# nv-nguyen/gigapose

Measured on NVIDIA H100. Metric: detections/sec (224x224 crops, 162-template bank), higher is better.
Workload: dtype f32 (a1, a4, a6: bf16 hi/lo split x3 on tensor cores with fp32 accumulate = fp32-faithful; a5, a7-a9: fp32)

## Files before the change

### gigapose_b200/csrc/gigapose_kernels.h

```cpp
#pragma once
#include <cuda_runtime.h>
#include <cuda.h>
#include <stdint.h>

namespace gp {

bool pdl_enabled();
template <typename... KArgs, typename... Args>
inline cudaError_t launch_ex(void (*kernel)(KArgs...), dim3 grid, dim3 block, size_t smem, cudaStream_t stream, int cluster_x,
                             bool pdl, Args&&... args) {
  cudaLaunchConfig_t cfg{};
  cfg.gridDim = grid; cfg.blockDim = block; cfg.dynamicSmemBytes = smem; cfg.stream = stream;
  cudaLaunchAttribute attr[2];
  int na = 0;
  if (cluster_x > 1) {
    attr[na].id = cudaLaunchAttributeClusterDimension;
    attr[na].val.clusterDim.x = cluster_x; attr[na].val.clusterDim.y = 1; attr[na].val.clusterDim.z = 1;
    ++na;
  }
  if (pdl && pdl_enabled()) {
    attr[na].id = cudaLaunchAttributeProgrammaticStreamSerialization;
    attr[na].val.programmaticStreamSerializationAllowed = 1;
    ++na;
  }
  cfg.attrs = attr; cfg.numAttrs = na;
  return cudaLaunchKernelEx(&cfg, kernel, static_cast<KArgs>(args)...);
}

struct SimSearchParams {
  int num_items;
  int B;
  int T;
  const int* perm;
  const int* q_obj;
  const float* q_mask;
  const float* bank_mask;
  float sim_threshold;
  float patch_threshold;
  int passes;
  float* sim_avg;
  float* rec_score;
  uint8_t* rec_idx;
  uint8_t* rec_valid;
  float* debug_tile;
};
cudaError_t launch_sim_search(const CUtensorMap& q_hi, const CUtensorMap& q_lo, const CUtensorMap& t_hi,
                              const CUtensorMap& t_lo, const SimSearchParams& p, int num_sms, cudaStream_t stream);
int sim_search_smem_bytes();

struct TopkSelectParams {
  int B, T, k;
  int id_stride, id_offset;
  const float* sim_avg;
  const float* rec_score;
  const uint8_t* rec_idx;
  const uint8_t* rec_valid;
  float* cand_score;
  int* cand_id;
  float* cand_pts_score;
  uint8_t* cand_idx;
  uint8_t* cand_valid;
};
cudaError_t launch_topk_select(const TopkSelectParams& p, cudaStream_t stream);

struct TopkMergeParams {
  int B, k, G;
  size_t rank_stride_bytes;
  const float* cand_score;
  const int* cand_id;
  const float* cand_pts_score;
  const uint8_t* cand_idx;
  const uint8_t* cand_valid;
  const float* cand_rel_scale;
  const float* cand_rel_inplane;
  float* out_rel_scale;
  float* out_rel_inplane;
  long long* id_src;
  float* score_src;
  float* score_pts;
  long long* tar_pts;
  long long* src_pts;
};
cudaError_t launch_topk_merge_expand(const TopkMergeParams& p, cudaStream_t stream);

cudaError_t launch_split_descriptors(const float* x, long long n_rows, int C, int rows_per_img, long long img_stride,
                                     long long row_stride, long long chan_stride, int norm_passes,
                                     int tiled ,
                                     uint16_t* hi, uint16_t* lo, float* normalized_out ,
                                     cudaStream_t stream);
cudaError_t launch_sample_mask16(const float* mask, long long n, int H, int W, float* out, cudaStream_t stream);
cudaError_t launch_object_order(const int* q_obj, int B, int num_objects, int* q_obj_out, int* perm, cudaStream_t stream);
cudaError_t launch_transpose_cp(const float* in, long long n, int C, float* out, cudaStream_t stream);

struct IstMlpWeights {
  const float *s_w1, *s_b1, *s_w2, *s_b2, *s_w3, *s_b3;
  const float *i_w1, *i_b1, *i_w2, *i_b2, *i_w3, *i_b3;
  int use_tanh;
};
struct IstMlpParams {
  int B, k;
  int T;
  int id_stride, id_offset;
  const long long* id_src;
  const long long* src_pts;
  const long long* tar_pts;
  const int* q_obj;
  const float* q_ist;
  const float* bank_ist;
  float* rel_scale;
  float* rel_inplane;
  int* row_count;
  int* row_ids;
  float* hidden1;
  float* hidden2;
};
cudaError_t launch_ist_mlp(const IstMlpWeights& w, const IstMlpParams& p, cudaStream_t stream);
cudaError_t launch_mlp_gather_planes(const IstMlpParams& p, uint16_t* a_hi, uint16_t* a_lo, cudaStream_t stream);
cudaError_t launch_mlp_head_rows(const IstMlpWeights& w, const IstMlpParams& p, const float* h2_scale, const float* h2_inplane,
                                 cudaStream_t stream);

struct RansacParams {
  int n;
  float pixel_threshold;
  int patch_size;
  const long long* src_pts;
  const long long* tar_pts;
  const float* rel_scale;
  const float* rel_inplane;
  float* M;
  uint8_t* failed;
  long long* in_src;
  long long* in_tar;
  long long* in_score;
  int* in_count;
};
cudaError_t launch_ransac(const RansacParams& p, cudaStream_t stream);

struct PoseParams {
  int B, k, T;
  int sort;
  const int* q_obj;
  const float* q_K;
  const float* q_M;
  const float* tmpl_K;
  const float* tmpl_M;
  const float* tmpl_pose;
  const int* in_count;
  const long long* id_src; const float* score_src; const float* score_pts;
  const long long* tar_pts; const long long* src_pts;
  const float* rel_scale; const float* rel_inplane;
  const float* M; const uint8_t* failed;
  const long long* in_src; const long long* in_tar; const long long* in_score;
  long long* o_id_src; float* o_score_src; float* o_score_pts;
  long long* o_tar_pts; long long* o_src_pts;
  float* o_rel_scale; float* o_rel_inplane;
  float* o_M; uint8_t* o_failed;
  long long* o_in_src; long long* o_in_tar; long long* o_in_score;
  float* o_scores;
  float* o_poses;
};
cudaError_t launch_sort_and_pose(const PoseParams& p, cudaStream_t stream);
cudaError_t launch_pose_only(int n, int k, int T, const int* q_obj, const float* q_K, const float* q_M,
                             const long long* id_src, const float* M, const float* tmpl_K, const float* tmpl_M,
                             const float* tmpl_pose, float* poses, cudaStream_t stream);

enum GemmMode { GEMM_PLANES = 0, GEMM_PLANES_GELU = 1, GEMM_SCALE_RESIDUAL = 2, GEMM_PATCH_EMBED = 3, GEMM_QKV_HEADS = 4,
                GEMM_PLANES_RELU = 5, GEMM_PLANES_ADD_RELU = 6, GEMM_ROWS_F32 = 7, GEMM_ROWS_F32_RELU = 8 };
struct GemmParams {
  int M, N, K;
  int passes;
  int mode;
  const float* bias;
  const float* gamma;
  float* x;
  uint16_t *out_hi, *out_lo;
  const float* pos;
  int tokens_per_img, patches_per_img;
  int qkv_crop_stride;
  int bn;
  int conv, Ho, Wo, stride, pad, kw, cblocks;
  int swap;
  const uint16_t *res_hi, *res_lo;
  const int* m_dev;
  float acc_scale;
  int f16;
  int stamp;
};
bool gemm_config_supported(const GemmParams& p, const char** why = nullptr);
cudaError_t launch_vit_gemm(const CUtensorMap& a_hi, const CUtensorMap& a_lo, const CUtensorMap& w_hi,
                            const CUtensorMap& w_lo, const GemmParams& p, int num_sms, cudaStream_t stream);
cudaError_t launch_split_planes(const float* x, long long rows, int K, int Kpad, uint16_t* hi, uint16_t* lo, cudaStream_t s,
                                bool f16 = false, float pre_scale = 1.0f);
cudaError_t launch_im2col(const float* img, int b, int Kpad, uint16_t* hi, uint16_t* lo, cudaStream_t s);
cudaError_t launch_cls_rows(const float* cls, const float* pos, int b, float* x, cudaStream_t s);
cudaError_t launch_layernorm_planes(const float* x, int M, const float* w, const float* b, float eps, uint16_t* hi,
                                    uint16_t* lo, cudaStream_t s);
cudaError_t launch_attention_tc(const CUtensorMap& hi128, const CUtensorMap& lo128, const CUtensorMap& hi16,
                                const CUtensorMap& lo16, const uint16_t* qkv_hi, const uint16_t* qkv_lo, uint16_t* out_hi,
                                uint16_t* out_lo, int b, int crop_stride, int passes, cudaStream_t s);
cudaError_t read_attention_stamps(long long* host32);
cudaError_t read_gemm_stamps(long long* host128);

}
```

### gigapose_b200/csrc/vit_api.cu

```cuda
#include "../../include/gigapose_b200.h"
#include "gigapose_kernels.h"

#include <cstdarg>
#include <cstdio>
#include <cstdlib>
#include <new>
#include <string>
#include <vector>

extern int gp_internal_fail(int code, const char* fmt, ...);
extern void gp_internal_count_launches(int n);
extern int gp_internal_make_map(CUtensorMap* map, void* ptr, uint64_t rows, uint64_t cols, uint32_t box_rows);
extern int gp_internal_make_map_ex(CUtensorMap* map, void* ptr, uint64_t rows, uint64_t cols, uint32_t box_cols,
                                   uint32_t box_rows, int swizzle_bytes);

namespace {

constexpr int kDim = 1024, kQkv = 3072, kMlp = 4096, kTok = 257, kPatchK = 588, kPatchKPad = 608;
constexpr float kLayerNormEps = 1e-6f;
constexpr size_t kAlign = 1024;
inline size_t up(size_t x) { return (x + kAlign - 1) / kAlign * kAlign; }

struct Carver {
  uint8_t* base; size_t off = 0;
  explicit Carver(void* b) : base(static_cast<uint8_t*>(b)) {}
  template <typename T> T* take(size_t n) { T* p = base ? reinterpret_cast<T*>(base + off) : nullptr; off += up(n * sizeof(T)); return p; }
};

struct Planes { uint16_t *hi, *lo; CUtensorMap m_hi, m_lo; };

struct BlockW {
  Planes qkv, proj, fc1, fc2;
  const float *n1w, *n1b, *qkv_b, *proj_b, *ls1, *n2w, *n2b, *fc1_b, *fc2_b, *ls2;
};

#define GPV_CUDA(expr)                                                                                    \
  do {                                                                                                    \
    cudaError_t _e = (expr);                                                                              \
    if (_e != cudaSuccess) return gp_internal_fail(GP_ERR_CUDA, "%s failed: %s", #expr, cudaGetErrorString(_e)); \
  } while (0)

}

struct gp_vit_context {
  int depth, max_crops, passes, num_sms;
  Planes patch_w;
  const float *patch_b, *cls, *pos;
  std::vector<BlockW> blocks;
  float* x;
  Planes ln, qkv, attn, hid, patches;
  CUtensorMap qkv_hi128, qkv_lo128, qkv_hi16, qkv_lo16;
  size_t workspace_bytes;
};

namespace {

void carve_weights(Carver& c, int depth, gp_vit_context* h) {
  auto planes = [&](Planes* p, size_t n) { uint16_t* a = c.take<uint16_t>(n); uint16_t* b = c.take<uint16_t>(n); if (p) { p->hi = a; p->lo = b; } };
  planes(h ? &h->patch_w : nullptr, (size_t)kDim * kPatchKPad);
  for (int i = 0; i < depth; ++i) {
    BlockW* b = h ? &h->blocks[i] : nullptr;
    planes(b ? &b->qkv : nullptr, (size_t)kQkv * kDim);
    planes(b ? &b->proj : nullptr, (size_t)kDim * kDim);
    planes(b ? &b->fc1 : nullptr, (size_t)kMlp * kDim);
    planes(b ? &b->fc2 : nullptr, (size_t)kDim * kMlp);
  }
}

void carve_workspace(Carver& c, int max_crops, gp_vit_context* h) {
  const size_t M = (size_t)max_crops * kTok;
  auto planes = [&](Planes* p, size_t n) { uint16_t* a = c.take<uint16_t>(n); uint16_t* b = c.take<uint16_t>(n); if (p) { p->hi = a; p->lo = b; } };
  float* x = c.take<float>(M * kDim);
  if (h) h->x = x;
  planes(h ? &h->ln : nullptr, M * kDim);
  planes(h ? &h->qkv : nullptr, M * kQkv);
  planes(h ? &h->attn : nullptr, M * kDim);
  planes(h ? &h->hid : nullptr, M * kMlp);
  planes(h ? &h->patches : nullptr, (size_t)max_crops * 256 * kPatchKPad);
}

int make_maps(Planes* p, uint64_t rows, uint64_t cols, uint32_t box_rows) {
  if (int e = gp_internal_make_map(&p->m_hi, p->hi, rows, cols, box_rows)) return e;
  return gp_internal_make_map(&p->m_lo, p->lo, rows, cols, box_rows);
}

}

extern "C" {

int gp_vit_query_sizes(int depth, int max_crops, size_t* weight_bytes, size_t* workspace_bytes) {
  if (depth < 1 || depth > 64 || max_crops < 1) return gp_internal_fail(GP_ERR_INVALID, "bad depth / max_crops");
  Carver cw(nullptr), cs(nullptr);
  carve_weights(cw, depth, nullptr);
  carve_workspace(cs, max_crops, nullptr);
  if (weight_bytes) *weight_bytes = cw.off;
  if (workspace_bytes) *workspace_bytes = cs.off;
  return GP_OK;
}

int gp_vit_create(int device, int depth, int max_crops, int precision, const float* const* w, void* weight_mem,
                  void* workspace_mem, void* stream, gp_vit_handle_t* out) {
  if (depth < 1 || depth > 64 || max_crops < 1 || !w || !weight_mem || !workspace_mem || !out)
    return gp_internal_fail(GP_ERR_INVALID, "bad argument");
  if (precision != GP_PRECISION_FP32_SPLIT && precision != GP_PRECISION_BF16)
    return gp_internal_fail(GP_ERR_INVALID, "unknown precision %d", precision);
  if (((uintptr_t)weight_mem | (uintptr_t)workspace_mem) & (kAlign - 1))
    return gp_internal_fail(GP_ERR_INVALID, "weight and workspace memory must be 1024-byte aligned");
  for (int i = 0; i < 4 + 14 * depth; ++i)
    if (!w[i]) return gp_internal_fail(GP_ERR_INVALID, "weight pointer %d is null", i);
  GPV_CUDA(cudaSetDevice(device));
  cudaDeviceProp prop;
  GPV_CUDA(cudaGetDeviceProperties(&prop, device));
  if (prop.major != 9 || prop.minor != 0) return gp_internal_fail(GP_ERR_UNSUPPORTED, "device %d is not sm_90", device);
  gp_vit_context* h = new (std::nothrow) gp_vit_context();
  if (!h) return gp_internal_fail(GP_ERR_INVALID, "out of host memory");
  h->depth = depth; h->max_crops = max_crops; h->num_sms = prop.multiProcessorCount;
  h->passes = precision == GP_PRECISION_FP32_SPLIT ? 3 : 1;
  h->blocks.resize(depth);
  Carver cw(weight_mem), cs(workspace_mem);
  carve_weights(cw, depth, h);
  carve_workspace(cs, max_crops, h);
  cudaStream_t s = static_cast<cudaStream_t>(stream);
  if (cudaMemsetAsync(workspace_mem, 0, cs.off, s) != cudaSuccess) { delete h; return gp_internal_fail(GP_ERR_CUDA, "workspace memset failed"); }

  h->patch_b = w[1]; h->cls = w[2]; h->pos = w[3];
  cudaError_t ce = gp::launch_split_planes(w[0], kDim, kPatchK, kPatchKPad, h->patch_w.hi, h->patch_w.lo, s);
  int e = ce == cudaSuccess ? make_maps(&h->patch_w, kDim, kPatchKPad, 256) : GP_ERR_CUDA;
  for (int i = 0; i < depth && !e && ce == cudaSuccess; ++i) {
    const float* const* b = w + 4 + 14 * i;
    BlockW& B = h->blocks[i];
    B.n1w = b[0]; B.n1b = b[1]; B.qkv_b = b[3]; B.proj_b = b[5]; B.ls1 = b[6];
    B.n2w = b[7]; B.n2b = b[8]; B.fc1_b = b[10]; B.fc2_b = b[12]; B.ls2 = b[13];
    if ((ce = gp::launch_split_planes(b[2], kQkv, kDim, kDim, B.qkv.hi, B.qkv.lo, s)) != cudaSuccess) break;
    if ((ce = gp::launch_split_planes(b[4], kDim, kDim, kDim, B.proj.hi, B.proj.lo, s)) != cudaSuccess) break;
    if ((ce = gp::launch_split_planes(b[9], kMlp, kDim, kDim, B.fc1.hi, B.fc1.lo, s)) != cudaSuccess) break;
    if ((ce = gp::launch_split_planes(b[11], kDim, kMlp, kMlp, B.fc2.hi, B.fc2.lo, s)) != cudaSuccess) break;
    if ((e = make_maps(&B.qkv, kQkv, kDim, 256)) || (e = make_maps(&B.proj, kDim, kDim, 256)) ||
        (e = make_maps(&B.fc1, kMlp, kDim, 256)) || (e = make_maps(&B.fc2, kDim, kMlp, 256)))
      break;
  }
  const uint64_t M = (uint64_t)max_crops * kTok;
  if (!e && ce == cudaSuccess)
    (e = make_maps(&h->ln, M, kDim, 128)) || (e = make_maps(&h->attn, M, kDim, 128)) || (e = make_maps(&h->hid, M, kMlp, 128)) ||
        (e = make_maps(&h->patches, (uint64_t)max_crops * 256, kPatchKPad, 128)) ||
        (e = gp_internal_make_map_ex(&h->qkv_hi128, h->qkv.hi, 48 * M, 64, 64, 128, 128)) ||
        (e = gp_internal_make_map_ex(&h->qkv_lo128, h->qkv.lo, 48 * M, 64, 64, 128, 128)) ||
        (e = gp_internal_make_map_ex(&h->qkv_hi16, h->qkv.hi, 48 * M, 64, 64, 16, 128)) ||
        (e = gp_internal_make_map_ex(&h->qkv_lo16, h->qkv.lo, 48 * M, 64, 64, 16, 128));
  if (ce != cudaSuccess) { delete h; return gp_internal_fail(GP_ERR_CUDA, "weight packing failed: %s", cudaGetErrorString(ce)); }
  if (e) { delete h; return e; }
  gp_internal_count_launches(1 + 4 * depth);
  *out = h;
  return GP_OK;
}

int gp_debug_attention_timeline(long long* stamps32) {
  if (!stamps32) return gp_internal_fail(GP_ERR_INVALID, "null argument");
  GPV_CUDA(cudaDeviceSynchronize());
  GPV_CUDA(gp::read_attention_stamps(stamps32));
  return GP_OK;
}

int gp_debug_gemm_timeline(long long* stamps128) {
  if (!stamps128) return gp_internal_fail(GP_ERR_INVALID, "null argument");
  GPV_CUDA(cudaDeviceSynchronize());
  GPV_CUDA(gp::read_gemm_stamps(stamps128));
  return GP_OK;
}

int gp_debug_gemm(const gp_debug_gemm_t* d, void* stream) {
  if (!d) return gp_internal_fail(GP_ERR_INVALID, "null argument");
  gp::GemmParams g{};
  g.M = d->M; g.N = d->N; g.K = d->K; g.bn = d->bn; g.passes = d->passes; g.mode = d->mode; g.swap = d->swap; g.f16 = d->f16;
  g.acc_scale = d->acc_scale; g.bias = d->bias; g.gamma = d->gamma; g.x = d->x; g.out_hi = d->out_hi; g.out_lo = d->out_lo;
  g.pos = d->pos; g.res_hi = d->res_hi; g.res_lo = d->res_lo; g.m_dev = d->m_dev;
  g.tokens_per_img = d->tokens_per_img; g.patches_per_img = d->patches_per_img; g.qkv_crop_stride = d->qkv_crop_stride;
  g.stamp = d->stamp;
  if (g.M < 1) return gp_internal_fail(GP_ERR_INVALID, "M must be >= 1");
  const char* why = nullptr;
  if (!gp::gemm_config_supported(g, &why)) return gp_internal_fail(GP_ERR_INVALID, "unsupported GEMM: %s", why);
  if (!d->a_hi || !d->a_lo || !d->w_hi || !d->w_lo || !d->bias) return gp_internal_fail(GP_ERR_INVALID, "null operand or bias");
  const bool planes_out = g.mode == gp::GEMM_PLANES || g.mode == gp::GEMM_PLANES_GELU || g.mode == gp::GEMM_QKV_HEADS ||
                          g.mode == gp::GEMM_PLANES_RELU || g.mode == gp::GEMM_PLANES_ADD_RELU;
  if (planes_out ? (!g.out_hi || !g.out_lo) : !g.x) return gp_internal_fail(GP_ERR_INVALID, "null output");
  if (g.mode == gp::GEMM_SCALE_RESIDUAL && !g.gamma) return gp_internal_fail(GP_ERR_INVALID, "null gamma");
  if (g.mode == gp::GEMM_PLANES_ADD_RELU && (!g.res_hi || !g.res_lo)) return gp_internal_fail(GP_ERR_INVALID, "null residual planes");
  if (g.mode == gp::GEMM_PATCH_EMBED && (!g.pos || g.patches_per_img < 1 || g.tokens_per_img <= g.patches_per_img))
    return gp_internal_fail(GP_ERR_INVALID, "patch embedding needs pos and tokens_per_img > patches_per_img >= 1");
  if (g.mode == gp::GEMM_QKV_HEADS && (g.N != kQkv || g.tokens_per_img < 1 || g.qkv_crop_stride * g.tokens_per_img < g.M))
    return gp_internal_fail(GP_ERR_INVALID, "QKV scatter needs N = 3072 and qkv_crop_stride * tokens_per_img >= M");
  if (g.swap && g.m_dev) return gp_internal_fail(GP_ERR_INVALID, "m_dev is not supported with swap");
  int dev = 0, sms = 0;
  GPV_CUDA(cudaGetDevice(&dev));
  GPV_CUDA(cudaDeviceGetAttribute(&sms, cudaDevAttrMultiProcessorCount, dev));
  const int bn = g.bn > 0 ? g.bn : 256;
  CUtensorMap a_hi, a_lo, w_hi, w_lo;
  auto* a_h = const_cast<uint16_t*>(d->a_hi); auto* a_l = const_cast<uint16_t*>(d->a_lo);
  auto* w_h = const_cast<uint16_t*>(d->w_hi); auto* w_l = const_cast<uint16_t*>(d->w_lo);
  if (int e = gp_internal_make_map(&a_hi, a_h, g.M, g.K, 128)) return e;
  if (int e = gp_internal_make_map(&a_lo, a_l, g.M, g.K, 128)) return e;
  if (int e = gp_internal_make_map(&w_hi, w_h, g.N, g.K, bn)) return e;
  if (int e = gp_internal_make_map(&w_lo, w_l, g.N, g.K, bn)) return e;
  GPV_CUDA(gp::launch_vit_gemm(a_hi, a_lo, w_hi, w_lo, g, sms, static_cast<cudaStream_t>(stream)));
  gp_internal_count_launches(1);
  return GP_OK;
}

int gp_debug_attention(int b, int crop_stride, int passes, const uint16_t* qkv_hi, const uint16_t* qkv_lo, uint16_t* out_hi,
                       uint16_t* out_lo, void* stream) {
  if (!qkv_hi || !qkv_lo || !out_hi || !out_lo) return gp_internal_fail(GP_ERR_INVALID, "null argument");
  if (b < 1 || crop_stride < b) return gp_internal_fail(GP_ERR_INVALID, "need 1 <= b (%d) <= crop_stride (%d)", b, crop_stride);
  if (passes != 1 && passes != 3) return gp_internal_fail(GP_ERR_INVALID, "passes must be 1 or 3");
  const uint64_t rows = 48ull * crop_stride * kTok;
  auto* qh = const_cast<uint16_t*>(qkv_hi); auto* ql = const_cast<uint16_t*>(qkv_lo);
  CUtensorMap hi128, lo128, hi16, lo16;
  if (int e = gp_internal_make_map_ex(&hi128, qh, rows, 64, 64, 128, 128)) return e;
  if (int e = gp_internal_make_map_ex(&lo128, ql, rows, 64, 64, 128, 128)) return e;
  if (int e = gp_internal_make_map_ex(&hi16, qh, rows, 64, 64, 16, 128)) return e;
  if (int e = gp_internal_make_map_ex(&lo16, ql, rows, 64, 64, 16, 128)) return e;
  GPV_CUDA(gp::launch_attention_tc(hi128, lo128, hi16, lo16, qkv_hi, qkv_lo, out_hi, out_lo, b, crop_stride, passes,
                                   static_cast<cudaStream_t>(stream)));
  gp_internal_count_launches(1);
  return GP_OK;
}

int gp_debug_layernorm(int M, const float* x, const float* w, const float* b, uint16_t* out_hi, uint16_t* out_lo,
                       void* stream) {
  if (!x || !w || !b || !out_hi || !out_lo) return gp_internal_fail(GP_ERR_INVALID, "null argument");
  if (M < 1) return gp_internal_fail(GP_ERR_INVALID, "M must be >= 1");
  GPV_CUDA(gp::launch_layernorm_planes(x, M, w, b, kLayerNormEps, out_hi, out_lo, static_cast<cudaStream_t>(stream)));
  gp_internal_count_launches(1);
  return GP_OK;
}

int gp_vit_destroy(gp_vit_handle_t h) {
  delete h;
  return GP_OK;
}

int gp_vit_time_linears(gp_vit_handle_t h, int b, int iters, float* avg_ms, void* stream) {
  if (!h || !avg_ms || iters < 1) return gp_internal_fail(GP_ERR_INVALID, "bad argument");
  if (b < 1 || b > h->max_crops) return gp_internal_fail(GP_ERR_INVALID, "batch %d outside [1, %d]", b, h->max_crops);
  cudaStream_t s = static_cast<cudaStream_t>(stream);
  const int M = b * kTok;
  auto linear = [&](const Planes& a, const Planes& w, gp::GemmParams& gp_) {
    return gp::launch_vit_gemm(a.m_hi, a.m_lo, w.m_hi, w.m_lo, gp_, h->num_sms, s);
  };
  auto run = [&]() -> int {
    for (int i = 0; i < h->depth; ++i) {
      const BlockW& B = h->blocks[i];
      gp::GemmParams g{};
      g.passes = h->passes; g.M = M; g.N = kQkv; g.K = kDim; g.mode = gp::GEMM_QKV_HEADS; g.bias = B.qkv_b;
      g.out_hi = h->qkv.hi; g.out_lo = h->qkv.lo; g.tokens_per_img = kTok; g.qkv_crop_stride = h->max_crops;
      GPV_CUDA(linear(h->ln, B.qkv, g));
      g = gp::GemmParams{}; g.passes = h->passes;
      g.M = M; g.N = kDim; g.K = kDim; g.mode = gp::GEMM_SCALE_RESIDUAL; g.bias = B.proj_b; g.gamma = B.ls1; g.x = h->x;
      GPV_CUDA(linear(h->attn, B.proj, g));
      g = gp::GemmParams{}; g.passes = h->passes;
      g.M = M; g.N = kMlp; g.K = kDim; g.mode = gp::GEMM_PLANES_GELU; g.bias = B.fc1_b; g.out_hi = h->hid.hi; g.out_lo = h->hid.lo;
      GPV_CUDA(linear(h->ln, B.fc1, g));
      g = gp::GemmParams{}; g.passes = h->passes;
      g.M = M; g.N = kDim; g.K = kMlp; g.mode = gp::GEMM_SCALE_RESIDUAL; g.bias = B.fc2_b; g.gamma = B.ls2; g.x = h->x;
      GPV_CUDA(linear(h->hid, B.fc2, g));
    }
    return GP_OK;
  };
  cudaEvent_t e0, e1;
  GPV_CUDA(cudaEventCreate(&e0));
  GPV_CUDA(cudaEventCreate(&e1));
  if (int e = run()) return e;
  GPV_CUDA(cudaEventRecord(e0, s));
  for (int it = 0; it < iters; ++it)
    if (int e = run()) return e;
  GPV_CUDA(cudaEventRecord(e1, s));
  GPV_CUDA(cudaEventSynchronize(e1));
  float ms = 0.f;
  GPV_CUDA(cudaEventElapsedTime(&ms, e0, e1));
  cudaEventDestroy(e0);
  cudaEventDestroy(e1);
  *avg_ms = ms / iters;
  gp_internal_count_launches(4 * h->depth * (iters + 1));
  return GP_OK;
}

int gp_vit_forward(gp_vit_handle_t h, int b, const float* img, float* x_prenorm, void* stream) {
  if (!h || !img || !x_prenorm) return gp_internal_fail(GP_ERR_INVALID, "null argument");
  if (b < 1 || b > h->max_crops) return gp_internal_fail(GP_ERR_INVALID, "batch %d outside [1, %d]", b, h->max_crops);
  cudaStream_t s = static_cast<cudaStream_t>(stream);
  const int M = b * kTok;
  GPV_CUDA(gp::launch_im2col(img, b, kPatchKPad, h->patches.hi, h->patches.lo, s));
  gp::GemmParams g{};
  g.passes = h->passes; g.tokens_per_img = kTok; g.patches_per_img = 256;
  g.M = b * 256; g.N = kDim; g.K = kPatchKPad; g.mode = gp::GEMM_PATCH_EMBED; g.bias = h->patch_b; g.pos = h->pos; g.x = h->x;
  GPV_CUDA(gp::launch_vit_gemm(h->patches.m_hi, h->patches.m_lo, h->patch_w.m_hi, h->patch_w.m_lo, g, h->num_sms, s));
  GPV_CUDA(gp::launch_cls_rows(h->cls, h->pos, b, h->x, s));
  auto linear = [&](const Planes& a, const Planes& w, gp::GemmParams& gp_) {
    return gp::launch_vit_gemm(a.m_hi, a.m_lo, w.m_hi, w.m_lo, gp_, h->num_sms, s);
  };
  for (int i = 0; i < h->depth; ++i) {
    const BlockW& B = h->blocks[i];
    GPV_CUDA(gp::launch_layernorm_planes(h->x, M, B.n1w, B.n1b, kLayerNormEps, h->ln.hi, h->ln.lo, s));
    g = gp::GemmParams{}; g.passes = h->passes;
    g.M = M; g.N = kQkv; g.K = kDim; g.mode = gp::GEMM_QKV_HEADS; g.bias = B.qkv_b; g.out_hi = h->qkv.hi; g.out_lo = h->qkv.lo;
    g.tokens_per_img = kTok; g.qkv_crop_stride = h->max_crops;
    GPV_CUDA(linear(h->ln, B.qkv, g));
    GPV_CUDA(gp::launch_attention_tc(h->qkv_hi128, h->qkv_lo128, h->qkv_hi16, h->qkv_lo16, h->qkv.hi, h->qkv.lo,
                                     h->attn.hi, h->attn.lo, b, h->max_crops, h->passes, s));
    g = gp::GemmParams{}; g.passes = h->passes;
    g.M = M; g.N = kDim; g.K = kDim; g.mode = gp::GEMM_SCALE_RESIDUAL; g.bias = B.proj_b; g.gamma = B.ls1; g.x = h->x;
    GPV_CUDA(linear(h->attn, B.proj, g));
    GPV_CUDA(gp::launch_layernorm_planes(h->x, M, B.n2w, B.n2b, kLayerNormEps, h->ln.hi, h->ln.lo, s));
    g = gp::GemmParams{}; g.passes = h->passes;
    g.M = M; g.N = kMlp; g.K = kDim; g.mode = gp::GEMM_PLANES_GELU; g.bias = B.fc1_b; g.out_hi = h->hid.hi; g.out_lo = h->hid.lo;
    GPV_CUDA(linear(h->ln, B.fc1, g));
    g = gp::GemmParams{}; g.passes = h->passes;
    g.M = M; g.N = kDim; g.K = kMlp; g.mode = gp::GEMM_SCALE_RESIDUAL; g.bias = B.fc2_b; g.gamma = B.ls2; g.x = h->x;
    GPV_CUDA(linear(h->hid, B.fc2, g));
  }
  GPV_CUDA(cudaMemcpyAsync(x_prenorm, h->x, (size_t)M * kDim * sizeof(float), cudaMemcpyDeviceToDevice, s));
  gp_internal_count_launches(3 + 7 * h->depth);
  return GP_OK;
}

}
```

### gigapose_b200/csrc/vit_attention_tc.cu

```cuda
#include "gigapose_kernels.h"
#include "common.cuh"
#include "wgmma.cuh"
#include <cuda_bf16.h>

namespace gp {

namespace {

constexpr int kTok = 257, kDim = 1024, kHeads = 16, kHd = 64;
constexpr int kKeys = 272;
constexpr int kRow = 128;
constexpr int kKVPlane = kKeys * kRow;
constexpr int kQPlane = 256 * kRow;
constexpr int kQTiles = 4;
constexpr int kMmaWarps = 8;
constexpr int kThreads = (kMmaWarps + 1) * 32;

struct __align__(8) AttnTail {
  uint64_t qk_full, v_full;
};
constexpr int kSmem = 1024 + 4 * kKVPlane + 2 * kQPlane + sizeof(AttnTail);

__device__ __forceinline__ void split_pair(float a, float b, uint32_t& hi, uint32_t& lo) {
  asm("cvt.rn.bf16x2.f32 %0, %1, %2;" : "=r"(hi) : "f"(b), "f"(a));
  const float ra = a - __uint_as_float(hi << 16), rb = b - __uint_as_float(hi & 0xffff0000u);
  asm("cvt.rn.bf16x2.f32 %0, %1, %2;" : "=r"(lo) : "f"(rb), "f"(ra));
}
__device__ __forceinline__ float ex2_approx(float x) {
  float y;
  asm("ex2.approx.ftz.f32 %0, %1;" : "=f"(y) : "f"(x));
  return y;
}
constexpr float kExpScale = 0.125f * 1.4426950408889634f;
__device__ __forceinline__ float2 ld_pair_sw128(const uint8_t* hi, const uint8_t* lo, int row, int col) {
  const uint32_t off = (uint32_t)row * 128u + ((((uint32_t)col >> 3) ^ ((uint32_t)row & 7u)) << 4) + (((uint32_t)col & 7u) << 1);
  const uint32_t h = *reinterpret_cast<const uint32_t*>(hi + off);
  const uint32_t l = lo ? *reinterpret_cast<const uint32_t*>(lo + off) : 0u;
  return make_float2(__uint_as_float(h << 16) + __uint_as_float(l << 16),
                     __uint_as_float(h & 0xffff0000u) + __uint_as_float(l & 0xffff0000u));
}

}

__device__ long long g_attn_stamp[32];
#define STAMP(i) do { if (blockIdx.x == 0) g_attn_stamp[i] = clock64(); } while (0)

template <int kPasses>
__global__ void __launch_bounds__(kThreads, 1)
attention_tc_kernel(const __grid_constant__ CUtensorMap tm_hi_128, const __grid_constant__ CUtensorMap tm_lo_128,
                    const __grid_constant__ CUtensorMap tm_hi_16, const __grid_constant__ CUtensorMap tm_lo_16,
                    const __nv_bfloat16* __restrict__ qkv_hi, const __nv_bfloat16* __restrict__ qkv_lo,
                    __nv_bfloat16* __restrict__ out_hi, __nv_bfloat16* __restrict__ out_lo, int crop_stride) {
  constexpr int passes = kPasses;
  constexpr int np = passes == 3 ? 2 : 1;
  extern __shared__ uint8_t smem_raw[];
  pdl_trigger();
  uint8_t* smem = smem_raw + ((1024u - (smem_u32(smem_raw) & 1023u)) & 1023u);
  uint8_t* sK[2] = {smem, smem + kKVPlane};
  uint8_t* sV[2] = {smem + 2 * kKVPlane, smem + 3 * kKVPlane};
  uint8_t* sQ[2] = {smem + 4 * kKVPlane, smem + 4 * kKVPlane + kQPlane};
  AttnTail& tail = *reinterpret_cast<AttnTail*>(smem + 4 * kKVPlane + 2 * kQPlane);
  const int warp = threadIdx.x >> 5, lane = threadIdx.x & 31;
  const int item = blockIdx.x;
  const int img = item / kHeads, head = item % kHeads;
  const int row0 = img * kTok;
  const int rq = ((0 * crop_stride + img) * kHeads + head) * kTok;
  const int rk = ((1 * crop_stride + img) * kHeads + head) * kTok;
  const int rv = ((2 * crop_stride + img) * kHeads + head) * kTok;

  if (threadIdx.x == 0) {
    mbar_init(&tail.qk_full, 1);
    mbar_init(&tail.v_full, 1);
    fence_barrier_init();
  }
  __syncthreads();
  pdl_wait();
  if (threadIdx.x == 0) STAMP(0);

  if (warp == kMmaWarps) {
    if (lane == 0) {
      tma_prefetch_desc(&tm_hi_128); tma_prefetch_desc(&tm_hi_16);
      if (np == 2) { tma_prefetch_desc(&tm_lo_128); tma_prefetch_desc(&tm_lo_16); }
      mbar_arrive_expect_tx(&tail.qk_full, (uint32_t)(np * (kQPlane + kKVPlane)));
      for (int pl = 0; pl < np; ++pl) {
        const CUtensorMap* m128 = pl ? &tm_lo_128 : &tm_hi_128;
        const CUtensorMap* m16 = pl ? &tm_lo_16 : &tm_hi_16;
        tma_load_2d(sQ[pl], m128, &tail.qk_full, 0, rq);
        tma_load_2d(sQ[pl] + 128 * kRow, m128, &tail.qk_full, 0, rq + 128);
        tma_load_2d(sK[pl], m128, &tail.qk_full, 0, rk);
        tma_load_2d(sK[pl] + 128 * kRow, m128, &tail.qk_full, 0, rk + 128);
        tma_load_2d(sK[pl] + 256 * kRow, m16, &tail.qk_full, 0, rk + 256);
      }
      mbar_arrive_expect_tx(&tail.v_full, (uint32_t)(np * kKVPlane));
      for (int pl = 0; pl < np; ++pl) {
        const CUtensorMap* m128 = pl ? &tm_lo_128 : &tm_hi_128;
        const CUtensorMap* m16 = pl ? &tm_lo_16 : &tm_hi_16;
        tma_load_2d(sV[pl], m128, &tail.v_full, 0, rv);
        tma_load_2d(sV[pl] + 128 * kRow, m128, &tail.v_full, 0, rv + 128);
        tma_load_2d(sV[pl] + 256 * kRow, m16, &tail.v_full, 0, rv + 256);
      }
    }
    __syncwarp();
    __shared__ float s_p[kKeys];
    __shared__ float s_q[kHd];
    {
    const size_t qoff = (size_t)(rq + 256) * kHd + 2 * lane;
    const uint32_t qh = *reinterpret_cast<const uint32_t*>(qkv_hi + qoff);
    const uint32_t ql = passes == 3 ? *reinterpret_cast<const uint32_t*>(qkv_lo + qoff) : 0u;
    s_q[2 * lane] = __uint_as_float(qh << 16) + __uint_as_float(ql << 16);
    s_q[2 * lane + 1] = __uint_as_float(qh & 0xffff0000u) + __uint_as_float(ql & 0xffff0000u);
    __syncwarp();
    mbar_wait(&tail.qk_full, 0);
    const uint8_t* klo = passes == 3 ? sK[1] : nullptr;
    const uint8_t* vlo = passes == 3 ? sV[1] : nullptr;
    float sj[9];
    float mx = -INFINITY;
#pragma unroll
    for (int i = 0; i < 9; ++i) {
      const int key = lane + 32 * i;
      float acc = 0.f;
      if (key < kTok) {
#pragma unroll
        for (int ch = 0; ch < 8; ++ch) {
          const uint32_t off = (uint32_t)key * 128u + (((uint32_t)ch ^ ((uint32_t)key & 7u)) << 4);
          const uint4 h4 = *reinterpret_cast<const uint4*>(sK[0] + off);
          const uint4 l4 = klo ? *reinterpret_cast<const uint4*>(klo + off) : make_uint4(0, 0, 0, 0);
          const uint32_t hw[4] = {h4.x, h4.y, h4.z, h4.w}, lw[4] = {l4.x, l4.y, l4.z, l4.w};
#pragma unroll
          for (int w = 0; w < 4; ++w) {
            const float k0 = __uint_as_float(hw[w] << 16) + __uint_as_float(lw[w] << 16);
            const float k1 = __uint_as_float(hw[w] & 0xffff0000u) + __uint_as_float(lw[w] & 0xffff0000u);
            acc = fmaf(s_q[ch * 8 + 2 * w], k0, acc);
            acc = fmaf(s_q[ch * 8 + 2 * w + 1], k1, acc);
          }
        }
      }
      sj[i] = key < kTok ? acc : -INFINITY;
      mx = fmaxf(mx, sj[i]);
    }
#pragma unroll
    for (int off = 16; off > 0; off >>= 1) mx = fmaxf(mx, __shfl_xor_sync(0xffffffffu, mx, off));
    float sum = 0.f;
#pragma unroll
    for (int i = 0; i < 9; ++i) {
      const int key = lane + 32 * i;
      const float pj = key < kTok ? ex2_approx((sj[i] - mx) * kExpScale) : 0.f;
      sum += pj;
      if (key < kKeys) s_p[key] = pj;
    }
#pragma unroll
    for (int off = 16; off > 0; off >>= 1) sum += __shfl_xor_sync(0xffffffffu, sum, off);
    __syncwarp();
    mbar_wait(&tail.v_full, 0);
    float o0[4] = {0.f, 0.f, 0.f, 0.f}, o1[4] = {0.f, 0.f, 0.f, 0.f};
#pragma unroll 8
    for (int key = 0; key < 256; ++key) {
      const float2 vv = ld_pair_sw128(sV[0], vlo, key, 2 * lane);
      const float pj = s_p[key];
      o0[key & 3] = fmaf(pj, vv.x, o0[key & 3]);
      o1[key & 3] = fmaf(pj, vv.y, o1[key & 3]);
    }
    {
      const float2 vv = ld_pair_sw128(sV[0], vlo, 256, 2 * lane);
      o0[0] = fmaf(s_p[256], vv.x, o0[0]);
      o1[0] = fmaf(s_p[256], vv.y, o1[0]);
    }
    const float o0s = (o0[0] + o0[1]) + (o0[2] + o0[3]), o1s = (o1[0] + o1[1]) + (o1[2] + o1[3]);
    const float inv = 1.0f / sum;
    uint32_t h, l;
    split_pair(o0s * inv, o1s * inv, h, l);
    const size_t oo = (size_t)(row0 + 256) * kDim + head * kHd + 2 * lane;
    *reinterpret_cast<uint32_t*>(out_hi + oo) = h;
    *reinterpret_cast<uint32_t*>(out_lo + oo) = l;
    }
  } else {
    const int wg = warp >> 2, wl = warp & 3;
    const uint32_t kh = smem_u32(sK[0]), kl = smem_u32(sK[1]), vh = smem_u32(sV[0]), vl = smem_u32(sV[1]);
    mbar_wait(&tail.qk_full, 0);
    if (threadIdx.x == 0) STAMP(1);
    for (int qt = wg; qt < kQTiles; qt += 2) {
      const uint32_t qh = smem_u32(sQ[0] + qt * 64 * kRow), ql = smem_u32(sQ[1] + qt * 64 * kRow);
      float s[128], st[8];
      acc_fence(s); acc_fence(st);
      wgmma_fence();
#pragma unroll
      for (int pass = 0; pass < passes; ++pass) {
        const uint32_t a = pass == 2 ? ql : qh, b = pass == 1 ? kl : kh;
#pragma unroll
        for (int k16 = 0; k16 < 4; ++k16) {
          const uint32_t acc = (pass | k16) != 0 ? 1u : 0u;
          const uint64_t da = wgmma_desc_kmajor<kRow>(a + k16 * 32);
          wgmma_ss_n256_bf16(s, da, wgmma_desc_kmajor<kRow>(b + k16 * 32), acc);
          wgmma_ss_n16_bf16(st, da, wgmma_desc_kmajor<kRow>(b + 256 * kRow + k16 * 32), acc);
        }
      }
      wgmma_commit();
      wgmma_wait<0>();
      acc_fence(s); acc_fence(st);
      const bool key256 = (lane & 3) == 0;
#pragma unroll
      for (int i = 0; i < 8; ++i) if (!(key256 && (i & 1) == 0 && i < 4)) st[i] = -INFINITY;
      float mx0 = fmaxf(st[0], st[1]), mx1 = fmaxf(st[2], st[3]);
#pragma unroll
      for (int j = 0; j < 32; ++j) {
        mx0 = fmaxf(mx0, fmaxf(s[4 * j], s[4 * j + 1]));
        mx1 = fmaxf(mx1, fmaxf(s[4 * j + 2], s[4 * j + 3]));
      }
#pragma unroll
      for (int off = 1; off <= 2; off <<= 1) {
        mx0 = fmaxf(mx0, __shfl_xor_sync(0xffffffffu, mx0, off));
        mx1 = fmaxf(mx1, __shfl_xor_sync(0xffffffffu, mx1, off));
      }
      float sum0 = 0.f, sum1 = 0.f;
      uint32_t ph[68], pl[68];
#pragma unroll
      for (int j = 0; j < 34; ++j) {
        const float x0 = j < 32 ? s[4 * j] : st[4 * (j - 32)], x1 = j < 32 ? s[4 * j + 1] : st[4 * (j - 32) + 1];
        const float x2 = j < 32 ? s[4 * j + 2] : st[4 * (j - 32) + 2], x3 = j < 32 ? s[4 * j + 3] : st[4 * (j - 32) + 3];
        const float p0 = ex2_approx((x0 - mx0) * kExpScale), p1 = ex2_approx((x1 - mx0) * kExpScale);
        const float p2 = ex2_approx((x2 - mx1) * kExpScale), p3 = ex2_approx((x3 - mx1) * kExpScale);
        sum0 += p0 + p1;
        sum1 += p2 + p3;
        const int c = j >> 1, h = (j & 1) * 2;
        split_pair(p0, p1, ph[4 * c + h], pl[4 * c + h]);
        split_pair(p2, p3, ph[4 * c + h + 1], pl[4 * c + h + 1]);
      }
#pragma unroll
      for (int off = 1; off <= 2; off <<= 1) {
        sum0 += __shfl_xor_sync(0xffffffffu, sum0, off);
        sum1 += __shfl_xor_sync(0xffffffffu, sum1, off);
      }
      if (qt == wg) mbar_wait(&tail.v_full, 0);
      float o[32];
      acc_fence(o);
      wgmma_fence();
#pragma unroll
      for (int c = 0; c < kKeys / 16; ++c) {
        const uint32_t ah[4] = {ph[4 * c], ph[4 * c + 1], ph[4 * c + 2], ph[4 * c + 3]};
        const uint64_t dvh = wgmma_desc_mnmajor_sw128(vh + c * 16 * kRow);
        wgmma_rs_n64_bf16_tb(o, ah, dvh, c != 0 ? 1u : 0u);
        if (passes == 3) {
          const uint32_t al[4] = {pl[4 * c], pl[4 * c + 1], pl[4 * c + 2], pl[4 * c + 3]};
          wgmma_rs_n64_bf16_tb(o, ah, wgmma_desc_mnmajor_sw128(vl + c * 16 * kRow), 1u);
          wgmma_rs_n64_bf16_tb(o, al, dvh, 1u);
        }
      }
      wgmma_commit();
      wgmma_wait<0>();
      acc_fence(o);
      const float inv0 = 1.0f / sum0, inv1 = 1.0f / sum1;
      const int tok0 = qt * 64 + wl * 16 + (lane >> 2);
      const size_t o0 = (size_t)(row0 + tok0) * kDim + head * kHd + 2 * (lane & 3);
      const size_t o1 = o0 + (size_t)8 * kDim;
#pragma unroll
      for (int j = 0; j < 8; ++j) {
        uint32_t h, l;
        split_pair(o[4 * j] * inv0, o[4 * j + 1] * inv0, h, l);
        *reinterpret_cast<uint32_t*>(out_hi + o0 + 8 * j) = h;
        *reinterpret_cast<uint32_t*>(out_lo + o0 + 8 * j) = l;
        split_pair(o[4 * j + 2] * inv1, o[4 * j + 3] * inv1, h, l);
        *reinterpret_cast<uint32_t*>(out_hi + o1 + 8 * j) = h;
        *reinterpret_cast<uint32_t*>(out_lo + o1 + 8 * j) = l;
      }
    }
    if (lane == 0 && wl == 0) STAMP(2 + wg);
  }
}

cudaError_t read_attention_stamps(long long* host32) {
  return cudaMemcpyFromSymbol(host32, g_attn_stamp, sizeof(long long) * 32);
}

cudaError_t launch_attention_tc(const CUtensorMap& hi128, const CUtensorMap& lo128, const CUtensorMap& hi16,
                                const CUtensorMap& lo16, const uint16_t* qkv_hi, const uint16_t* qkv_lo, uint16_t* out_hi,
                                uint16_t* out_lo, int b, int crop_stride, int passes, cudaStream_t s) {
  static bool configured = false;
  if (!configured) {
    cudaError_t e = cudaFuncSetAttribute(attention_tc_kernel<3>, cudaFuncAttributeMaxDynamicSharedMemorySize, kSmem);
    if (e == cudaSuccess) e = cudaFuncSetAttribute(attention_tc_kernel<1>, cudaFuncAttributeMaxDynamicSharedMemorySize, kSmem);
    if (e != cudaSuccess) return e;
    configured = true;
  }
  if (b <= 0) return cudaSuccess;
  const int items = b * kHeads;
  const dim3 grid(items);
  auto qh = reinterpret_cast<const __nv_bfloat16*>(qkv_hi), ql = reinterpret_cast<const __nv_bfloat16*>(qkv_lo);
  auto oh = reinterpret_cast<__nv_bfloat16*>(out_hi), ol = reinterpret_cast<__nv_bfloat16*>(out_lo);
  if (passes == 3)
    return launch_ex(attention_tc_kernel<3>, grid, dim3(kThreads), kSmem, s, 1, true, hi128, lo128, hi16, lo16, qh, ql, oh, ol, crop_stride);
  return launch_ex(attention_tc_kernel<1>, grid, dim3(kThreads), kSmem, s, 1, true, hi128, lo128, hi16, lo16, qh, ql, oh, ol, crop_stride);
}

}
```

### gigapose_b200/csrc/wgmma.cuh

```cuda
#pragma once
#include <stdint.h>

namespace gp {

__device__ __forceinline__ void wgmma_ss_n16_bf16(float (&d)[8], uint64_t da, uint64_t db, uint32_t scale_d) {
  asm volatile(
      "{\n\t.reg .pred p;\n\t"
      "setp.ne.b32 p, %10, 0;\n\t"
      "wgmma.mma_async.sync.aligned.m64n16k16.f32.bf16.bf16 "
      "{%0, %1, %2, %3, %4, %5, %6, %7}, "
      "%8, %9, p, 1, 1, 0, 0;\n\t}"
      : "+f"(d[0]), "+f"(d[1]), "+f"(d[2]), "+f"(d[3]), "+f"(d[4]), "+f"(d[5]), "+f"(d[6]), "+f"(d[7])
      : "l"(da), "l"(db), "r"(scale_d));
}
__device__ __forceinline__ void wgmma_ss_n16_f16(float (&d)[8], uint64_t da, uint64_t db, uint32_t scale_d) {
  asm volatile(
      "{\n\t.reg .pred p;\n\t"
      "setp.ne.b32 p, %10, 0;\n\t"
      "wgmma.mma_async.sync.aligned.m64n16k16.f32.f16.f16 "
      "{%0, %1, %2, %3, %4, %5, %6, %7}, "
      "%8, %9, p, 1, 1, 0, 0;\n\t}"
      : "+f"(d[0]), "+f"(d[1]), "+f"(d[2]), "+f"(d[3]), "+f"(d[4]), "+f"(d[5]), "+f"(d[6]), "+f"(d[7])
      : "l"(da), "l"(db), "r"(scale_d));
}
__device__ __forceinline__ void wgmma_ss_n64_bf16(float (&d)[32], uint64_t da, uint64_t db, uint32_t scale_d) {
  asm volatile(
      "{\n\t.reg .pred p;\n\t"
      "setp.ne.b32 p, %34, 0;\n\t"
      "wgmma.mma_async.sync.aligned.m64n64k16.f32.bf16.bf16 "
      "{%0, %1, %2, %3, %4, %5, %6, %7, %8, %9, %10, %11, %12, %13, %14, %15, %16, %17, %18, %19, %20, %21, %22, %23, %24, %25, %26, %27, %28, %29, %30, %31}, "
      "%32, %33, p, 1, 1, 0, 0;\n\t}"
      : "+f"(d[0]), "+f"(d[1]), "+f"(d[2]), "+f"(d[3]), "+f"(d[4]), "+f"(d[5]), "+f"(d[6]), "+f"(d[7]), "+f"(d[8]), "+f"(d[9]), "+f"(d[10]), "+f"(d[11]), "+f"(d[12]), "+f"(d[13]), "+f"(d[14]), "+f"(d[15]), "+f"(d[16]), "+f"(d[17]), "+f"(d[18]), "+f"(d[19]), "+f"(d[20]), "+f"(d[21]), "+f"(d[22]), "+f"(d[23]), "+f"(d[24]), "+f"(d[25]), "+f"(d[26]), "+f"(d[27]), "+f"(d[28]), "+f"(d[29]), "+f"(d[30]), "+f"(d[31])
      : "l"(da), "l"(db), "r"(scale_d));
}
__device__ __forceinline__ void wgmma_ss_n64_f16(float (&d)[32], uint64_t da, uint64_t db, uint32_t scale_d) {
  asm volatile(
      "{\n\t.reg .pred p;\n\t"
      "setp.ne.b32 p, %34, 0;\n\t"
      "wgmma.mma_async.sync.aligned.m64n64k16.f32.f16.f16 "
      "{%0, %1, %2, %3, %4, %5, %6, %7, %8, %9, %10, %11, %12, %13, %14, %15, %16, %17, %18, %19, %20, %21, %22, %23, %24, %25, %26, %27, %28, %29, %30, %31}, "
      "%32, %33, p, 1, 1, 0, 0;\n\t}"
      : "+f"(d[0]), "+f"(d[1]), "+f"(d[2]), "+f"(d[3]), "+f"(d[4]), "+f"(d[5]), "+f"(d[6]), "+f"(d[7]), "+f"(d[8]), "+f"(d[9]), "+f"(d[10]), "+f"(d[11]), "+f"(d[12]), "+f"(d[13]), "+f"(d[14]), "+f"(d[15]), "+f"(d[16]), "+f"(d[17]), "+f"(d[18]), "+f"(d[19]), "+f"(d[20]), "+f"(d[21]), "+f"(d[22]), "+f"(d[23]), "+f"(d[24]), "+f"(d[25]), "+f"(d[26]), "+f"(d[27]), "+f"(d[28]), "+f"(d[29]), "+f"(d[30]), "+f"(d[31])
      : "l"(da), "l"(db), "r"(scale_d));
}
__device__ __forceinline__ void wgmma_ss_n192_bf16(float (&d)[96], uint64_t da, uint64_t db, uint32_t scale_d) {
  asm volatile(
      "{\n\t.reg .pred p;\n\t"
      "setp.ne.b32 p, %98, 0;\n\t"
      "wgmma.mma_async.sync.aligned.m64n192k16.f32.bf16.bf16 "
      "{%0, %1, %2, %3, %4, %5, %6, %7, %8, %9, %10, %11, %12, %13, %14, %15, %16, %17, %18, %19, %20, %21, %22, %23, %24, %25, %26, %27, %28, %29, %30, %31, %32, %33, %34, %35, %36, %37, %38, %39, %40, %41, %42, %43, %44, %45, %46, %47, %48, %49, %50, %51, %52, %53, %54, %55, %56, %57, %58, %59, %60, %61, %62, %63, %64, %65, %66, %67, %68, %69, %70, %71, %72, %73, %74, %75, %76, %77, %78, %79, %80, %81, %82, %83, %84, %85, %86, %87, %88, %89, %90, %91, %92, %93, %94, %95}, "
      "%96, %97, p, 1, 1, 0, 0;\n\t}"
      : "+f"(d[0]), "+f"(d[1]), "+f"(d[2]), "+f"(d[3]), "+f"(d[4]), "+f"(d[5]), "+f"(d[6]), "+f"(d[7]), "+f"(d[8]), "+f"(d[9]), "+f"(d[10]), "+f"(d[11]), "+f"(d[12]), "+f"(d[13]), "+f"(d[14]), "+f"(d[15]), "+f"(d[16]), "+f"(d[17]), "+f"(d[18]), "+f"(d[19]), "+f"(d[20]), "+f"(d[21]), "+f"(d[22]), "+f"(d[23]), "+f"(d[24]), "+f"(d[25]), "+f"(d[26]), "+f"(d[27]), "+f"(d[28]), "+f"(d[29]), "+f"(d[30]), "+f"(d[31]), "+f"(d[32]), "+f"(d[33]), "+f"(d[34]), "+f"(d[35]), "+f"(d[36]), "+f"(d[37]), "+f"(d[38]), "+f"(d[39]), "+f"(d[40]), "+f"(d[41]), "+f"(d[42]), "+f"(d[43]), "+f"(d[44]), "+f"(d[45]), "+f"(d[46]), "+f"(d[47]), "+f"(d[48]), "+f"(d[49]), "+f"(d[50]), "+f"(d[51]), "+f"(d[52]), "+f"(d[53]), "+f"(d[54]), "+f"(d[55]), "+f"(d[56]), "+f"(d[57]), "+f"(d[58]), "+f"(d[59]), "+f"(d[60]), "+f"(d[61]), "+f"(d[62]), "+f"(d[63]), "+f"(d[64]), "+f"(d[65]), "+f"(d[66]), "+f"(d[67]), "+f"(d[68]), "+f"(d[69]), "+f"(d[70]), "+f"(d[71]), "+f"(d[72]), "+f"(d[73]), "+f"(d[74]), "+f"(d[75]), "+f"(d[76]), "+f"(d[77]), "+f"(d[78]), "+f"(d[79]), "+f"(d[80]), "+f"(d[81]), "+f"(d[82]), "+f"(d[83]), "+f"(d[84]), "+f"(d[85]), "+f"(d[86]), "+f"(d[87]), "+f"(d[88]), "+f"(d[89]), "+f"(d[90]), "+f"(d[91]), "+f"(d[92]), "+f"(d[93]), "+f"(d[94]), "+f"(d[95])
      : "l"(da), "l"(db), "r"(scale_d));
}
__device__ __forceinline__ void wgmma_ss_n192_f16(float (&d)[96], uint64_t da, uint64_t db, uint32_t scale_d) {
  asm volatile(
      "{\n\t.reg .pred p;\n\t"
      "setp.ne.b32 p, %98, 0;\n\t"
      "wgmma.mma_async.sync.aligned.m64n192k16.f32.f16.f16 "
      "{%0, %1, %2, %3, %4, %5, %6, %7, %8, %9, %10, %11, %12, %13, %14, %15, %16, %17, %18, %19, %20, %21, %22, %23, %24, %25, %26, %27, %28, %29, %30, %31, %32, %33, %34, %35, %36, %37, %38, %39, %40, %41, %42, %43, %44, %45, %46, %47, %48, %49, %50, %51, %52, %53, %54, %55, %56, %57, %58, %59, %60, %61, %62, %63, %64, %65, %66, %67, %68, %69, %70, %71, %72, %73, %74, %75, %76, %77, %78, %79, %80, %81, %82, %83, %84, %85, %86, %87, %88, %89, %90, %91, %92, %93, %94, %95}, "
      "%96, %97, p, 1, 1, 0, 0;\n\t}"
      : "+f"(d[0]), "+f"(d[1]), "+f"(d[2]), "+f"(d[3]), "+f"(d[4]), "+f"(d[5]), "+f"(d[6]), "+f"(d[7]), "+f"(d[8]), "+f"(d[9]), "+f"(d[10]), "+f"(d[11]), "+f"(d[12]), "+f"(d[13]), "+f"(d[14]), "+f"(d[15]), "+f"(d[16]), "+f"(d[17]), "+f"(d[18]), "+f"(d[19]), "+f"(d[20]), "+f"(d[21]), "+f"(d[22]), "+f"(d[23]), "+f"(d[24]), "+f"(d[25]), "+f"(d[26]), "+f"(d[27]), "+f"(d[28]), "+f"(d[29]), "+f"(d[30]), "+f"(d[31]), "+f"(d[32]), "+f"(d[33]), "+f"(d[34]), "+f"(d[35]), "+f"(d[36]), "+f"(d[37]), "+f"(d[38]), "+f"(d[39]), "+f"(d[40]), "+f"(d[41]), "+f"(d[42]), "+f"(d[43]), "+f"(d[44]), "+f"(d[45]), "+f"(d[46]), "+f"(d[47]), "+f"(d[48]), "+f"(d[49]), "+f"(d[50]), "+f"(d[51]), "+f"(d[52]), "+f"(d[53]), "+f"(d[54]), "+f"(d[55]), "+f"(d[56]), "+f"(d[57]), "+f"(d[58]), "+f"(d[59]), "+f"(d[60]), "+f"(d[61]), "+f"(d[62]), "+f"(d[63]), "+f"(d[64]), "+f"(d[65]), "+f"(d[66]), "+f"(d[67]), "+f"(d[68]), "+f"(d[69]), "+f"(d[70]), "+f"(d[71]), "+f"(d[72]), "+f"(d[73]), "+f"(d[74]), "+f"(d[75]), "+f"(d[76]), "+f"(d[77]), "+f"(d[78]), "+f"(d[79]), "+f"(d[80]), "+f"(d[81]), "+f"(d[82]), "+f"(d[83]), "+f"(d[84]), "+f"(d[85]), "+f"(d[86]), "+f"(d[87]), "+f"(d[88]), "+f"(d[89]), "+f"(d[90]), "+f"(d[91]), "+f"(d[92]), "+f"(d[93]), "+f"(d[94]), "+f"(d[95])
      : "l"(da), "l"(db), "r"(scale_d));
}
__device__ __forceinline__ void wgmma_ss_n256_bf16(float (&d)[128], uint64_t da, uint64_t db, uint32_t scale_d) {
  asm volatile(
      "{\n\t.reg .pred p;\n\t"
      "setp.ne.b32 p, %130, 0;\n\t"
      "wgmma.mma_async.sync.aligned.m64n256k16.f32.bf16.bf16 "
      "{%0, %1, %2, %3, %4, %5, %6, %7, %8, %9, %10, %11, %12, %13, %14, %15, %16, %17, %18, %19, %20, %21, %22, %23, %24, %25, %26, %27, %28, %29, %30, %31, %32, %33, %34, %35, %36, %37, %38, %39, %40, %41, %42, %43, %44, %45, %46, %47, %48, %49, %50, %51, %52, %53, %54, %55, %56, %57, %58, %59, %60, %61, %62, %63, %64, %65, %66, %67, %68, %69, %70, %71, %72, %73, %74, %75, %76, %77, %78, %79, %80, %81, %82, %83, %84, %85, %86, %87, %88, %89, %90, %91, %92, %93, %94, %95, %96, %97, %98, %99, %100, %101, %102, %103, %104, %105, %106, %107, %108, %109, %110, %111, %112, %113, %114, %115, %116, %117, %118, %119, %120, %121, %122, %123, %124, %125, %126, %127}, "
      "%128, %129, p, 1, 1, 0, 0;\n\t}"
      : "+f"(d[0]), "+f"(d[1]), "+f"(d[2]), "+f"(d[3]), "+f"(d[4]), "+f"(d[5]), "+f"(d[6]), "+f"(d[7]), "+f"(d[8]), "+f"(d[9]), "+f"(d[10]), "+f"(d[11]), "+f"(d[12]), "+f"(d[13]), "+f"(d[14]), "+f"(d[15]), "+f"(d[16]), "+f"(d[17]), "+f"(d[18]), "+f"(d[19]), "+f"(d[20]), "+f"(d[21]), "+f"(d[22]), "+f"(d[23]), "+f"(d[24]), "+f"(d[25]), "+f"(d[26]), "+f"(d[27]), "+f"(d[28]), "+f"(d[29]), "+f"(d[30]), "+f"(d[31]), "+f"(d[32]), "+f"(d[33]), "+f"(d[34]), "+f"(d[35]), "+f"(d[36]), "+f"(d[37]), "+f"(d[38]), "+f"(d[39]), "+f"(d[40]), "+f"(d[41]), "+f"(d[42]), "+f"(d[43]), "+f"(d[44]), "+f"(d[45]), "+f"(d[46]), "+f"(d[47]), "+f"(d[48]), "+f"(d[49]), "+f"(d[50]), "+f"(d[51]), "+f"(d[52]), "+f"(d[53]), "+f"(d[54]), "+f"(d[55]), "+f"(d[56]), "+f"(d[57]), "+f"(d[58]), "+f"(d[59]), "+f"(d[60]), "+f"(d[61]), "+f"(d[62]), "+f"(d[63]), "+f"(d[64]), "+f"(d[65]), "+f"(d[66]), "+f"(d[67]), "+f"(d[68]), "+f"(d[69]), "+f"(d[70]), "+f"(d[71]), "+f"(d[72]), "+f"(d[73]), "+f"(d[74]), "+f"(d[75]), "+f"(d[76]), "+f"(d[77]), "+f"(d[78]), "+f"(d[79]), "+f"(d[80]), "+f"(d[81]), "+f"(d[82]), "+f"(d[83]), "+f"(d[84]), "+f"(d[85]), "+f"(d[86]), "+f"(d[87]), "+f"(d[88]), "+f"(d[89]), "+f"(d[90]), "+f"(d[91]), "+f"(d[92]), "+f"(d[93]), "+f"(d[94]), "+f"(d[95]), "+f"(d[96]), "+f"(d[97]), "+f"(d[98]), "+f"(d[99]), "+f"(d[100]), "+f"(d[101]), "+f"(d[102]), "+f"(d[103]), "+f"(d[104]), "+f"(d[105]), "+f"(d[106]), "+f"(d[107]), "+f"(d[108]), "+f"(d[109]), "+f"(d[110]), "+f"(d[111]), "+f"(d[112]), "+f"(d[113]), "+f"(d[114]), "+f"(d[115]), "+f"(d[116]), "+f"(d[117]), "+f"(d[118]), "+f"(d[119]), "+f"(d[120]), "+f"(d[121]), "+f"(d[122]), "+f"(d[123]), "+f"(d[124]), "+f"(d[125]), "+f"(d[126]), "+f"(d[127])
      : "l"(da), "l"(db), "r"(scale_d));
}
__device__ __forceinline__ void wgmma_ss_n256_f16(float (&d)[128], uint64_t da, uint64_t db, uint32_t scale_d) {
  asm volatile(
      "{\n\t.reg .pred p;\n\t"
      "setp.ne.b32 p, %130, 0;\n\t"
      "wgmma.mma_async.sync.aligned.m64n256k16.f32.f16.f16 "
      "{%0, %1, %2, %3, %4, %5, %6, %7, %8, %9, %10, %11, %12, %13, %14, %15, %16, %17, %18, %19, %20, %21, %22, %23, %24, %25, %26, %27, %28, %29, %30, %31, %32, %33, %34, %35, %36, %37, %38, %39, %40, %41, %42, %43, %44, %45, %46, %47, %48, %49, %50, %51, %52, %53, %54, %55, %56, %57, %58, %59, %60, %61, %62, %63, %64, %65, %66, %67, %68, %69, %70, %71, %72, %73, %74, %75, %76, %77, %78, %79, %80, %81, %82, %83, %84, %85, %86, %87, %88, %89, %90, %91, %92, %93, %94, %95, %96, %97, %98, %99, %100, %101, %102, %103, %104, %105, %106, %107, %108, %109, %110, %111, %112, %113, %114, %115, %116, %117, %118, %119, %120, %121, %122, %123, %124, %125, %126, %127}, "
      "%128, %129, p, 1, 1, 0, 0;\n\t}"
      : "+f"(d[0]), "+f"(d[1]), "+f"(d[2]), "+f"(d[3]), "+f"(d[4]), "+f"(d[5]), "+f"(d[6]), "+f"(d[7]), "+f"(d[8]), "+f"(d[9]), "+f"(d[10]), "+f"(d[11]), "+f"(d[12]), "+f"(d[13]), "+f"(d[14]), "+f"(d[15]), "+f"(d[16]), "+f"(d[17]), "+f"(d[18]), "+f"(d[19]), "+f"(d[20]), "+f"(d[21]), "+f"(d[22]), "+f"(d[23]), "+f"(d[24]), "+f"(d[25]), "+f"(d[26]), "+f"(d[27]), "+f"(d[28]), "+f"(d[29]), "+f"(d[30]), "+f"(d[31]), "+f"(d[32]), "+f"(d[33]), "+f"(d[34]), "+f"(d[35]), "+f"(d[36]), "+f"(d[37]), "+f"(d[38]), "+f"(d[39]), "+f"(d[40]), "+f"(d[41]), "+f"(d[42]), "+f"(d[43]), "+f"(d[44]), "+f"(d[45]), "+f"(d[46]), "+f"(d[47]), "+f"(d[48]), "+f"(d[49]), "+f"(d[50]), "+f"(d[51]), "+f"(d[52]), "+f"(d[53]), "+f"(d[54]), "+f"(d[55]), "+f"(d[56]), "+f"(d[57]), "+f"(d[58]), "+f"(d[59]), "+f"(d[60]), "+f"(d[61]), "+f"(d[62]), "+f"(d[63]), "+f"(d[64]), "+f"(d[65]), "+f"(d[66]), "+f"(d[67]), "+f"(d[68]), "+f"(d[69]), "+f"(d[70]), "+f"(d[71]), "+f"(d[72]), "+f"(d[73]), "+f"(d[74]), "+f"(d[75]), "+f"(d[76]), "+f"(d[77]), "+f"(d[78]), "+f"(d[79]), "+f"(d[80]), "+f"(d[81]), "+f"(d[82]), "+f"(d[83]), "+f"(d[84]), "+f"(d[85]), "+f"(d[86]), "+f"(d[87]), "+f"(d[88]), "+f"(d[89]), "+f"(d[90]), "+f"(d[91]), "+f"(d[92]), "+f"(d[93]), "+f"(d[94]), "+f"(d[95]), "+f"(d[96]), "+f"(d[97]), "+f"(d[98]), "+f"(d[99]), "+f"(d[100]), "+f"(d[101]), "+f"(d[102]), "+f"(d[103]), "+f"(d[104]), "+f"(d[105]), "+f"(d[106]), "+f"(d[107]), "+f"(d[108]), "+f"(d[109]), "+f"(d[110]), "+f"(d[111]), "+f"(d[112]), "+f"(d[113]), "+f"(d[114]), "+f"(d[115]), "+f"(d[116]), "+f"(d[117]), "+f"(d[118]), "+f"(d[119]), "+f"(d[120]), "+f"(d[121]), "+f"(d[122]), "+f"(d[123]), "+f"(d[124]), "+f"(d[125]), "+f"(d[126]), "+f"(d[127])
      : "l"(da), "l"(db), "r"(scale_d));
}
__device__ __forceinline__ void wgmma_rs_n64_bf16_tb(float (&d)[32], const uint32_t (&a)[4], uint64_t db, uint32_t scale_d) {
  asm volatile(
      "{\n\t.reg .pred p;\n\t"
      "setp.ne.b32 p, %37, 0;\n\t"
      "wgmma.mma_async.sync.aligned.m64n64k16.f32.bf16.bf16 "
      "{%0, %1, %2, %3, %4, %5, %6, %7, %8, %9, %10, %11, %12, %13, %14, %15, %16, %17, %18, %19, %20, %21, %22, %23, %24, %25, %26, %27, %28, %29, %30, %31}, "
      "{%32, %33, %34, %35}, %36, p, 1, 1, 1;\n\t}"
      : "+f"(d[0]), "+f"(d[1]), "+f"(d[2]), "+f"(d[3]), "+f"(d[4]), "+f"(d[5]), "+f"(d[6]), "+f"(d[7]), "+f"(d[8]), "+f"(d[9]), "+f"(d[10]), "+f"(d[11]), "+f"(d[12]), "+f"(d[13]), "+f"(d[14]), "+f"(d[15]), "+f"(d[16]), "+f"(d[17]), "+f"(d[18]), "+f"(d[19]), "+f"(d[20]), "+f"(d[21]), "+f"(d[22]), "+f"(d[23]), "+f"(d[24]), "+f"(d[25]), "+f"(d[26]), "+f"(d[27]), "+f"(d[28]), "+f"(d[29]), "+f"(d[30]), "+f"(d[31])
      : "r"(a[0]), "r"(a[1]), "r"(a[2]), "r"(a[3]), "l"(db), "r"(scale_d));
}

__device__ __forceinline__ void wgmma_fence() { asm volatile("wgmma.fence.sync.aligned;" ::: "memory"); }
__device__ __forceinline__ void wgmma_commit() { asm volatile("wgmma.commit_group.sync.aligned;" ::: "memory"); }
template <int kPending>
__device__ __forceinline__ void wgmma_wait() { asm volatile("wgmma.wait_group.sync.aligned %0;" ::"n"(kPending) : "memory"); }
template <int kN>
__device__ __forceinline__ void acc_fence(float (&d)[kN]) {
#pragma unroll
  for (int i = 0; i < kN; ++i) asm volatile("" : "+f"(d[i])::"memory");
}

}
```

Before: 800.2.

## Make ViT attention kernel persistent with warp-specialized K/V pipeline and register rebalancing

Converts the attention kernel from one CTA per (image, head) into a persistent grid capped at the SM count. Each CTA loops over items, with a producer warp streaming K and V through full/empty mbarriers and setmaxnreg splitting registers between producer and consumer warpgroups. Q is no longer staged through shared memory, which shrinks the smem footprint. The aim is to cut launch and tail overhead and overlap TMA loads of the next item with compute on the current one. The cost is more barrier handshaking, and per-CTA throughput now depends on a single CTA per SM.

```diff
diff --git a/gigapose_b200/csrc/gigapose_kernels.h b/gigapose_b200/csrc/gigapose_kernels.h
--- a/gigapose_b200/csrc/gigapose_kernels.h
+++ b/gigapose_b200/csrc/gigapose_kernels.h
@@ -197,7 +197,7 @@
                                     uint16_t* lo, cudaStream_t s);
 cudaError_t launch_attention_tc(const CUtensorMap& hi128, const CUtensorMap& lo128, const CUtensorMap& hi16,
                                 const CUtensorMap& lo16, const uint16_t* qkv_hi, const uint16_t* qkv_lo, uint16_t* out_hi,
-                                uint16_t* out_lo, int b, int crop_stride, int passes, cudaStream_t s);
+                                uint16_t* out_lo, int b, int crop_stride, int passes, int num_sms, cudaStream_t s);
 cudaError_t read_attention_stamps(long long* host32);
 cudaError_t read_gemm_stamps(long long* host128);
 
diff --git a/gigapose_b200/csrc/vit_api.cu b/gigapose_b200/csrc/vit_api.cu
--- a/gigapose_b200/csrc/vit_api.cu
+++ b/gigapose_b200/csrc/vit_api.cu
@@ -218,7 +218,10 @@
   if (int e = gp_internal_make_map_ex(&lo128, ql, rows, 64, 64, 128, 128)) return e;
   if (int e = gp_internal_make_map_ex(&hi16, qh, rows, 64, 64, 16, 128)) return e;
   if (int e = gp_internal_make_map_ex(&lo16, ql, rows, 64, 64, 16, 128)) return e;
-  GPV_CUDA(gp::launch_attention_tc(hi128, lo128, hi16, lo16, qkv_hi, qkv_lo, out_hi, out_lo, b, crop_stride, passes,
+  int dev = 0, sms = 0;
+  GPV_CUDA(cudaGetDevice(&dev));
+  GPV_CUDA(cudaDeviceGetAttribute(&sms, cudaDevAttrMultiProcessorCount, dev));
+  GPV_CUDA(gp::launch_attention_tc(hi128, lo128, hi16, lo16, qkv_hi, qkv_lo, out_hi, out_lo, b, crop_stride, passes, sms,
                                    static_cast<cudaStream_t>(stream)));
   gp_internal_count_launches(1);
   return GP_OK;
@@ -305,7 +308,7 @@
     g.tokens_per_img = kTok; g.qkv_crop_stride = h->max_crops;
     GPV_CUDA(linear(h->ln, B.qkv, g));
     GPV_CUDA(gp::launch_attention_tc(h->qkv_hi128, h->qkv_lo128, h->qkv_hi16, h->qkv_lo16, h->qkv.hi, h->qkv.lo,
-                                     h->attn.hi, h->attn.lo, b, h->max_crops, h->passes, s));
+                                     h->attn.hi, h->attn.lo, b, h->max_crops, h->passes, h->num_sms, s));
     g = gp::GemmParams{}; g.passes = h->passes;
     g.M = M; g.N = kDim; g.K = kDim; g.mode = gp::GEMM_SCALE_RESIDUAL; g.bias = B.proj_b; g.gamma = B.ls1; g.x = h->x;
     GPV_CUDA(linear(h->attn, B.proj, g));
diff --git a/gigapose_b200/csrc/vit_attention_tc.cu b/gigapose_b200/csrc/vit_attention_tc.cu
--- a/gigapose_b200/csrc/vit_attention_tc.cu
+++ b/gigapose_b200/csrc/vit_attention_tc.cu
@@ -11,15 +11,18 @@
 constexpr int kKeys = 272;
 constexpr int kRow = 128;
 constexpr int kKVPlane = kKeys * kRow;
-constexpr int kQPlane = 256 * kRow;
-constexpr int kQTiles = 4;
-constexpr int kMmaWarps = 8;
-constexpr int kThreads = (kMmaWarps + 1) * 32;
+constexpr int kThreads = 3 * 128;
+constexpr int kKEmptyArrivals = 8 + 3;
+constexpr int kVEmptyArrivals = 8 + 2;
+constexpr int kTokBarrier = 1, kTokThreads = 96;
+constexpr int kPvBarrier = 2, kPvThreads = 64;
+constexpr uint32_t kProducerRegs = 40, kConsumerRegs = 232;
+static_assert(128 * kProducerRegs + 256 * kConsumerRegs <= 168 * kThreads, "register pool of the CTA");
 
 struct __align__(8) AttnTail {
-  uint64_t qk_full, v_full;
+  uint64_t k_full, k_empty, v_full, v_empty;
 };
-constexpr int kSmem = 1024 + 4 * kKVPlane + 2 * kQPlane + sizeof(AttnTail);
+constexpr int kSmem = 1024 + 4 * kKVPlane + sizeof(AttnTail);
 
 __device__ __forceinline__ void split_pair(float a, float b, uint32_t& hi, uint32_t& lo) {
   asm("cvt.rn.bf16x2.f32 %0, %1, %2;" : "=r"(hi) : "f"(b), "f"(a));
@@ -32,25 +35,54 @@
   return y;
 }
 constexpr float kExpScale = 0.125f * 1.4426950408889634f;
-__device__ __forceinline__ float2 ld_pair_sw128(const uint8_t* hi, const uint8_t* lo, int row, int col) {
-  const uint32_t off = (uint32_t)row * 128u + ((((uint32_t)col >> 3) ^ ((uint32_t)row & 7u)) << 4) + (((uint32_t)col & 7u) << 1);
-  const uint32_t h = *reinterpret_cast<const uint32_t*>(hi + off);
-  const uint32_t l = lo ? *reinterpret_cast<const uint32_t*>(lo + off) : 0u;
-  return make_float2(__uint_as_float(h << 16) + __uint_as_float(l << 16),
-                     __uint_as_float(h & 0xffff0000u) + __uint_as_float(l & 0xffff0000u));
-}
-
-}
-
+__device__ __forceinline__ void load_q_frag(uint32_t (&f)[16], const __nv_bfloat16* q) {
+  const uint32_t* p = reinterpret_cast<const uint32_t*>(q);
+#pragma unroll
+  for (int k = 0; k < 4; ++k) {
+    f[4 * k] = __ldg(p + 8 * k);
+    f[4 * k + 1] = __ldg(p + 8 * k + 4 * kHd);
+    f[4 * k + 2] = __ldg(p + 8 * k + 4);
+    f[4 * k + 3] = __ldg(p + 8 * k + 4 * kHd + 4);
+  }
+}
+__device__ __forceinline__ int cta_id() {
+  int x;
+  asm volatile("mov.u32 %0, %%ctaid.x;" : "=r"(x));
+  return x;
+}
+__device__ __forceinline__ int opaque(int x) {
+  asm volatile("" : "+r"(x));
+  return x;
+}
+__device__ __forceinline__ int n_cta() {
+  int x;
+  asm volatile("mov.u32 %0, %%nctaid.x;" : "=r"(x));
+  return x;
+}
+__device__ __forceinline__ uint2 lds_v2(uint32_t addr) {
+  uint2 v;
+  asm volatile("ld.shared.v2.u32 {%0, %1}, [%2];" : "=r"(v.x), "=r"(v.y) : "r"(addr));
+  return v;
+}
+__device__ __forceinline__ float lds_f32(uint32_t addr) {
+  float v;
+  asm volatile("ld.shared.f32 %0, [%1];" : "=f"(v) : "r"(addr));
+  return v;
+}
+__device__ __forceinline__ void prefetch_l2(const void* p) { asm volatile("prefetch.global.L2 [%0];" ::"l"(p)); }
+
+}
+
+constexpr int kStampItems = 5;
 __device__ long long g_attn_stamp[32];
-#define STAMP(i) do { if (blockIdx.x == 0) g_attn_stamp[i] = clock64(); } while (0)
+#define STAMP(i) (g_attn_stamp[i] = clock64())
 
 template <int kPasses>
 __global__ void __launch_bounds__(kThreads, 1)
 attention_tc_kernel(const __grid_constant__ CUtensorMap tm_hi_128, const __grid_constant__ CUtensorMap tm_lo_128,
                     const __grid_constant__ CUtensorMap tm_hi_16, const __grid_constant__ CUtensorMap tm_lo_16,
                     const __nv_bfloat16* __restrict__ qkv_hi, const __nv_bfloat16* __restrict__ qkv_lo,
-                    __nv_bfloat16* __restrict__ out_hi, __nv_bfloat16* __restrict__ out_lo, int crop_stride) {
+                    __nv_bfloat16* __restrict__ out_hi, __nv_bfloat16* __restrict__ out_lo, int crop_stride, int items) {
   constexpr int passes = kPasses;
   constexpr int np = passes == 3 ? 2 : 1;
   extern __shared__ uint8_t smem_raw[];
@@ -58,212 +90,309 @@
   uint8_t* smem = smem_raw + ((1024u - (smem_u32(smem_raw) & 1023u)) & 1023u);
   uint8_t* sK[2] = {smem, smem + kKVPlane};
   uint8_t* sV[2] = {smem + 2 * kKVPlane, smem + 3 * kKVPlane};
-  uint8_t* sQ[2] = {smem + 4 * kKVPlane, smem + 4 * kKVPlane + kQPlane};
-  AttnTail& tail = *reinterpret_cast<AttnTail*>(smem + 4 * kKVPlane + 2 * kQPlane);
+  AttnTail& tail = *reinterpret_cast<AttnTail*>(smem + 4 * kKVPlane);
   const int warp = threadIdx.x >> 5, lane = threadIdx.x & 31;
-  const int item = blockIdx.x;
-  const int img = item / kHeads, head = item % kHeads;
-  const int row0 = img * kTok;
-  const int rq = ((0 * crop_stride + img) * kHeads + head) * kTok;
-  const int rk = ((1 * crop_stride + img) * kHeads + head) * kTok;
-  const int rv = ((2 * crop_stride + img) * kHeads + head) * kTok;
+  auto plane_row = [&](int which, int item) { return ((which * crop_stride + item / kHeads) * kHeads + item % kHeads) * kTok; };
 
   if (threadIdx.x == 0) {
-    mbar_init(&tail.qk_full, 1);
+    mbar_init(&tail.k_full, 1);
     mbar_init(&tail.v_full, 1);
+    mbar_init(&tail.k_empty, kKEmptyArrivals);
+    mbar_init(&tail.v_empty, kVEmptyArrivals);
     fence_barrier_init();
   }
   __syncthreads();
   pdl_wait();
-  if (threadIdx.x == 0) STAMP(0);
-
-  if (warp == kMmaWarps) {
-    if (lane == 0) {
+  if (threadIdx.x == 0 && blockIdx.x == 0) STAMP(0);
+
+  if (warp < 4) {
+    setmaxnreg_dec<kProducerRegs>();
+    if (warp == 0 && lane == 0) {
       tma_prefetch_desc(&tm_hi_128); tma_prefetch_desc(&tm_hi_16);
       if (np == 2) { tma_prefetch_desc(&tm_lo_128); tma_prefetch_desc(&tm_lo_16); }
-      mbar_arrive_expect_tx(&tail.qk_full, (uint32_t)(np * (kQPlane + kKVPlane)));
-      for (int pl = 0; pl < np; ++pl) {
-        const CUtensorMap* m128 = pl ? &tm_lo_128 : &tm_hi_128;
-        const CUtensorMap* m16 = pl ? &tm_lo_16 : &tm_hi_16;
-        tma_load_2d(sQ[pl], m128, &tail.qk_full, 0, rq);
-        tma_load_2d(sQ[pl] + 128 * kRow, m128, &tail.qk_full, 0, rq + 128);
-        tma_load_2d(sK[pl], m128, &tail.qk_full, 0, rk);
-        tma_load_2d(sK[pl] + 128 * kRow, m128, &tail.qk_full, 0, rk + 128);
-        tma_load_2d(sK[pl] + 256 * kRow, m16, &tail.qk_full, 0, rk + 256);
+      uint32_t it = 0;
+      for (int item = cta_id(); item < items; item += gridDim.x, ++it) {
+        const int rk = plane_row(1, item), rv = plane_row(2, item);
+        if (it > 0) mbar_wait(&tail.k_empty, (it - 1) & 1);
+        mbar_arrive_expect_tx(&tail.k_full, (uint32_t)(np * kKVPlane));
+        for (int pl = 0; pl < np; ++pl) {
+          const CUtensorMap* m128 = pl ? &tm_lo_128 : &tm_hi_128;
+          const CUtensorMap* m16 = pl ? &tm_lo_16 : &tm_hi_16;
+          tma_load_2d(sK[pl], m128, &tail.k_full, 0, rk);
+          tma_load_2d(sK[pl] + 128 * kRow, m128, &tail.k_full, 0, rk + 128);
+          tma_load_2d(sK[pl] + 256 * kRow, m16, &tail.k_full, 0, rk + 256);
+        }
+        if (it > 0) mbar_wait(&tail.v_empty, (it - 1) & 1);
+        mbar_arrive_expect_tx(&tail.v_full, (uint32_t)(np * kKVPlane));
+        for (int pl = 0; pl < np; ++pl) {
+          const CUtensorMap* m128 = pl ? &tm_lo_128 : &tm_hi_128;
+          const CUtensorMap* m16 = pl ? &tm_lo_16 : &tm_hi_16;
+          tma_load_2d(sV[pl], m128, &tail.v_full, 0, rv);
+          tma_load_2d(sV[pl] + 128 * kRow, m128, &tail.v_full, 0, rv + 128);
+          tma_load_2d(sV[pl] + 256 * kRow, m16, &tail.v_full, 0, rv + 256);
+        }
       }
-      mbar_arrive_expect_tx(&tail.v_full, (uint32_t)(np * kKVPlane));
-      for (int pl = 0; pl < np; ++pl) {
-        const CUtensorMap* m128 = pl ? &tm_lo_128 : &tm_hi_128;
-        const CUtensorMap* m16 = pl ? &tm_lo_16 : &tm_hi_16;
-        tma_load_2d(sV[pl], m128, &tail.v_full, 0, rv);
-        tma_load_2d(sV[pl] + 128 * kRow, m128, &tail.v_full, 0, rv + 128);
-        tma_load_2d(sV[pl] + 256 * kRow, m16, &tail.v_full, 0, rv + 256);
+    } else if (warp > 0) {
+      __shared__ float s_p[kKeys];
+      __shared__ __align__(16) float s_q[kHd];
+      __shared__ __align__(16) float s_o[4][kHd];
+      const int tw = warp - 1;
+      uint32_t it = 0;
+      for (int item = cta_id(); item < items; item += n_cta(), ++it) {
+        const uint32_t ph = it & 1;
+        named_barrier_sync(kTokBarrier, kTokThreads);
+        if (tw == 0) {
+          const size_t qoff = (size_t)(plane_row(0, item) + 256) * kHd + 2 * lane;
+          const uint32_t qh = *reinterpret_cast<const uint32_t*>(qkv_hi + qoff);
+          const uint32_t ql = passes == 3 ? *reinterpret_cast<const uint32_t*>(qkv_lo + qoff) : 0u;
+          s_q[2 * lane] = __uint_as_float(qh << 16) + __uint_as_float(ql << 16);
+          s_q[2 * lane + 1] = __uint_as_float(qh & 0xffff0000u) + __uint_as_float(ql & 0xffff0000u);
+        }
+        named_barrier_sync(kTokBarrier, kTokThreads);
+        mbar_wait(&tail.k_full, ph);
+        if (tw == 0 && lane == 0 && cta_id() == 0 && it < kStampItems) STAMP(21 + 2 * it);
+        float sj[3] = {0.f, 0.f, 0.f};
+#pragma unroll 1
+        for (int ch = 0; ch < 8; ++ch) {
+          const float4 qa = *reinterpret_cast<const float4*>(s_q + ch * 8), qb = *reinterpret_cast<const float4*>(s_q + ch * 8 + 4);
+          const float q8[8] = {qa.x, qa.y, qa.z, qa.w, qb.x, qb.y, qb.z, qb.w};
+          const uint32_t off = (uint32_t)lane * 128u + (((uint32_t)ch ^ ((uint32_t)lane & 7u)) << 4);
+#pragma unroll
+          for (int j = 0; j < 3; ++j) {
+            const int i = tw + 3 * j;
+            if (lane + 32 * i < kTok) {
+              const uint4 h4 = *reinterpret_cast<const uint4*>(sK[0] + off + i * 32 * kRow);
+              const uint4 l4 = passes == 3 ? *reinterpret_cast<const uint4*>(sK[1] + off + i * 32 * kRow) : make_uint4(0, 0, 0, 0);
+              const uint32_t hw[4] = {h4.x, h4.y, h4.z, h4.w}, lw[4] = {l4.x, l4.y, l4.z, l4.w};
+#pragma unroll
+              for (int w = 0; w < 4; ++w) {
+                const float k0 = __uint_as_float(hw[w] << 16) + __uint_as_float(lw[w] << 16);
+                const float k1 = __uint_as_float(hw[w] & 0xffff0000u) + __uint_as_float(lw[w] & 0xffff0000u);
+                sj[j] = fmaf(q8[2 * w], k0, sj[j]);
+                sj[j] = fmaf(q8[2 * w + 1], k1, sj[j]);
+              }
+            }
+          }
+        }
+        __syncwarp();
+        if (lane == 0) mbar_arrive(&tail.k_empty);
+#pragma unroll
+        for (int j = 0; j < 3; ++j) {
+          const int key = opaque(lane) + 32 * (tw + 3 * j);
+          if (key < kKeys) s_p[key] = key < kTok ? sj[j] : -INFINITY;
+        }
+        named_barrier_sync(kTokBarrier, kTokThreads);
+        float sum = 0.f;
+        if (tw == 0) {
+          float mx = -INFINITY;
+#pragma unroll
+          for (int i = 0; i < 9; ++i) {
+            const int key = lane + 32 * i;
+            if (key < kTok) mx = fmaxf(mx, s_p[key]);
+          }
+#pragma unroll
+          for (int off = 16; off > 0; off >>= 1) mx = fmaxf(mx, __shfl_xor_sync(0xffffffffu, mx, off));
+#pragma unroll
+          for (int i = 0; i < 9; ++i) {
+            const int key = lane + 32 * i;
+            if (key < kKeys) {
+              const float pj = key < kTok ? ex2_approx((s_p[key] - mx) * kExpScale) : 0.f;
+              sum += pj;
+              s_p[key] = pj;
+            }
+          }
+#pragma unroll
+          for (int off = 16; off > 0; off >>= 1) sum += __shfl_xor_sync(0xffffffffu, sum, off);
+        }
+        named_barrier_sync(kTokBarrier, kTokThreads);
+        if (tw == 2) continue;
+        mbar_wait(&tail.v_full, opaque(it) & 1);
+        const int c = tw * 2 + (lane >> 4), qd = lane & 15;
+        const uint32_t col = (((uint32_t)qd >> 1) << 4), colb = ((uint32_t)qd & 1u) << 3;
+        float acc[4] = {0.f, 0.f, 0.f, 0.f};
+#pragma unroll 1
+        for (int k16 = 0; k16 < 256; k16 += 16) {
+          uint2 vh4[4], vl4[4];
+          float pk[4];
+#pragma unroll
+          for (int j = 0; j < 4; ++j) {
+            const int key = k16 + 4 * j + c;
+            const uint32_t off = (uint32_t)key * 128u + (col ^ (((uint32_t)key & 7u) << 4)) + colb;
+            vh4[j] = lds_v2(smem_u32(sV[0]) + off);
+            vl4[j] = passes == 3 ? lds_v2(smem_u32(sV[1]) + off) : make_uint2(0u, 0u);
+            pk[j] = lds_f32(smem_u32(s_p) + 4u * (uint32_t)key);
+          }
+#pragma unroll
+          for (int j = 0; j < 4; ++j) {
+            const uint32_t hw[2] = {vh4[j].x, vh4[j].y}, lw[2] = {vl4[j].x, vl4[j].y};
+#pragma unroll
+            for (int w = 0; w < 2; ++w) {
+              acc[2 * w] = fmaf(pk[j], __uint_as_float(hw[w] << 16) + __uint_as_float(lw[w] << 16), acc[2 * w]);
+              acc[2 * w + 1] = fmaf(pk[j], __uint_as_float(hw[w] & 0xffff0000u) + __uint_as_float(lw[w] & 0xffff0000u),
+                                    acc[2 * w + 1]);
+            }
+          }
+        }
+        const int ln = opaque(lane);
+        if (c == 0) {
+          const uint32_t off = 256u * 128u + (((uint32_t)(ln & 15) >> 1) << 4) + (((uint32_t)ln & 1u) << 3);
+          const uint2 h4 = *reinterpret_cast<const uint2*>(sV[0] + off);
+          const uint2 l4 = passes == 3 ? *reinterpret_cast<const uint2*>(sV[1] + off) : make_uint2(0u, 0u);
+          const uint32_t hw[2] = {h4.x, h4.y}, lw[2] = {l4.x, l4.y};
+          const float p256 = s_p[256];
+#pragma unroll
+          for (int w = 0; w < 2; ++w) {
+            acc[2 * w] = fmaf(p256, __uint_as_float(hw[w] << 16) + __uint_as_float(lw[w] << 16), acc[2 * w]);
+            acc[2 * w + 1] = fmaf(p256, __uint_as_float(hw[w] & 0xffff0000u) + __uint_as_float(lw[w] & 0xffff0000u),
+                                  acc[2 * w + 1]);
+          }
+        }
+        __syncwarp();
+        if (lane == 0) mbar_arrive(&tail.v_empty);
+        *reinterpret_cast<float4*>(&s_o[c][4 * (ln & 15)]) = make_float4(acc[0], acc[1], acc[2], acc[3]);
+        named_barrier_sync(kPvBarrier, kPvThreads);
+        if (tw == 1) continue;
+        const float2 a0 = *reinterpret_cast<const float2*>(&s_o[0][2 * lane]), a1 = *reinterpret_cast<const float2*>(&s_o[1][2 * lane]);
+        const float2 a2 = *reinterpret_cast<const float2*>(&s_o[2][2 * lane]), a3 = *reinterpret_cast<const float2*>(&s_o[3][2 * lane]);
+        const float o0s = (a0.x + a1.x) + (a2.x + a3.x), o1s = (a0.y + a1.y) + (a2.y + a3.y);
+        const float inv = 1.0f / sum;
+        uint32_t h, l;
+        split_pair(o0s * inv, o1s * inv, h, l);
+        const int oi = opaque(item);
+        const size_t oo = (size_t)((oi / kHeads) * kTok + 256) * kDim + (oi % kHeads) * kHd + 2 * lane;
+        *reinterpret_cast<uint32_t*>(out_hi + oo) = h;
+        *reinterpret_cast<uint32_t*>(out_lo + oo) = l;
+        if (lane == 0 && cta_id() == 0 && it < kStampItems) STAMP(22 + 2 * it);
       }
     }
-    __syncwarp();
-    __shared__ float s_p[kKeys];
-    __shared__ float s_q[kHd];
-    {
-    const size_t qoff = (size_t)(rq + 256) * kHd + 2 * lane;
-    const uint32_t qh = *reinterpret_cast<const uint32_t*>(qkv_hi + qoff);
-    const uint32_t ql = passes == 3 ? *reinterpret_cast<const uint32_t*>(qkv_lo + qoff) : 0u;
-    s_q[2 * lane] = __uint_as_float(qh << 16) + __uint_as_float(ql << 16);
-    s_q[2 * lane + 1] = __uint_as_float(qh & 0xffff0000u) + __uint_as_float(ql & 0xffff0000u);
-    __syncwarp();
-    mbar_wait(&tail.qk_full, 0);
-    const uint8_t* klo = passes == 3 ? sK[1] : nullptr;
-    const uint8_t* vlo = passes == 3 ? sV[1] : nullptr;
-    float sj[9];
-    float mx = -INFINITY;
-#pragma unroll
-    for (int i = 0; i < 9; ++i) {
-      const int key = lane + 32 * i;
-      float acc = 0.f;
-      if (key < kTok) {
-#pragma unroll
-        for (int ch = 0; ch < 8; ++ch) {
-          const uint32_t off = (uint32_t)key * 128u + (((uint32_t)ch ^ ((uint32_t)key & 7u)) << 4);
-          const uint4 h4 = *reinterpret_cast<const uint4*>(sK[0] + off);
-          const uint4 l4 = klo ? *reinterpret_cast<const uint4*>(klo + off) : make_uint4(0, 0, 0, 0);
-          const uint32_t hw[4] = {h4.x, h4.y, h4.z, h4.w}, lw[4] = {l4.x, l4.y, l4.z, l4.w};
-#pragma unroll
-          for (int w = 0; w < 4; ++w) {
-            const float k0 = __uint_as_float(hw[w] << 16) + __uint_as_float(lw[w] << 16);
-            const float k1 = __uint_as_float(hw[w] & 0xffff0000u) + __uint_as_float(lw[w] & 0xffff0000u);
-            acc = fmaf(s_q[ch * 8 + 2 * w], k0, acc);
-            acc = fmaf(s_q[ch * 8 + 2 * w + 1], k1, acc);
-          }
+  } else {
+    setmaxnreg_inc<kConsumerRegs>();
+    const int wg = (warp - 4) >> 2, wl = (warp - 4) & 3;
+    const uint32_t kh = smem_u32(sK[0]), kl = smem_u32(sK[1]), vh = smem_u32(sV[0]), vl = smem_u32(sV[1]);
+    const int cta = cta_id();
+    const bool stamp = threadIdx.x == 128 && cta == 0;
+    const int qfrag = (wl * 16 + (lane >> 2)) * kHd + 2 * (lane & 3);
+    auto q_at = [&](int item, int qt) { return (size_t)(plane_row(0, item) + qt * 64) * kHd + qfrag; };
+    uint32_t qa_h[16], qa_l[16];
+    load_q_frag(qa_h, qkv_hi + q_at(cta, wg));
+    if (passes == 3) load_q_frag(qa_l, qkv_lo + q_at(cta, wg));
+    uint32_t it = 0;
+    for (int item = cta; item < items; item += gridDim.x, ++it) {
+      const uint32_t ph = it & 1;
+      const int row0 = (item / kHeads) * kTok, head = item % kHeads;
+      if (stamp && it < kStampItems) STAMP(1 + 4 * it);
+      mbar_wait(&tail.k_full, ph);
+      if (stamp && it < kStampItems) STAMP(2 + 4 * it);
+#pragma unroll 1
+      for (int u = 0; u < 2; ++u) {
+        const int qt = wg + 2 * u;
+        float s[128], st[8];
+        acc_fence(s); acc_fence(st);
+        wgmma_fence();
+#pragma unroll
+        for (int pass = 0; pass < passes; ++pass) {
+          const uint32_t b = pass == 1 ? kl : kh;
+#pragma unroll
+          for (int k16 = 0; k16 < 4; ++k16) {
+            const uint32_t acc = (pass | k16) != 0 ? 1u : 0u;
+            const uint32_t a[4] = {pass == 2 ? qa_l[4 * k16] : qa_h[4 * k16], pass == 2 ? qa_l[4 * k16 + 1] : qa_h[4 * k16 + 1],
+                                   pass == 2 ? qa_l[4 * k16 + 2] : qa_h[4 * k16 + 2], pass == 2 ? qa_l[4 * k16 + 3] : qa_h[4 * k16 + 3]};
+            wgmma_rs_n256_bf16(s, a, wgmma_desc_kmajor<kRow>(b + k16 * 32), acc);
+            wgmma_rs_n16_bf16(st, a, wgmma_desc_kmajor<kRow>(b + 256 * kRow + k16 * 32), acc);
+          }
+        }
+        wgmma_commit();
+        wgmma_wait<0>();
+        acc_fence(s); acc_fence(st);
+        if (u == 1) {
+          __syncwarp();
+          if (lane == 0) mbar_arrive(&tail.k_empty);
+        }
+        const int nitem = u == 0 ? item : item + gridDim.x;
+        const size_t qnext = nitem < items ? q_at(nitem, u == 0 ? qt + 2 : wg) : 0;
+        if (nitem < items) {
+          load_q_frag(qa_h, qkv_hi + qnext);
+          if (passes == 3) {
+            prefetch_l2(qkv_lo + qnext);
+            prefetch_l2(qkv_lo + qnext + 8 * kHd);
+          }
+        }
+        const bool key256 = (lane & 3) == 0;
+#pragma unroll
+        for (int i = 0; i < 8; ++i) if (!(key256 && (i & 1) == 0 && i < 4)) st[i] = -INFINITY;
+        float mx0 = fmaxf(st[0], st[1]), mx1 = fmaxf(st[2], st[3]);
+#pragma unroll
+        for (int j = 0; j < 32; ++j) {
+          mx0 = fmaxf(mx0, fmaxf(s[4 * j], s[4 * j + 1]));
+          mx1 = fmaxf(mx1, fmaxf(s[4 * j + 2], s[4 * j + 3]));
+        }
+#pragma unroll
+        for (int off = 1; off <= 2; off <<= 1) {
+          mx0 = fmaxf(mx0, __shfl_xor_sync(0xffffffffu, mx0, off));
+          mx1 = fmaxf(mx1, __shfl_xor_sync(0xffffffffu, mx1, off));
+        }
+        float sum0 = 0.f, sum1 = 0.f;
+        uint32_t ph_[68], pl_[68];
+#pragma unroll
+        for (int j = 0; j < 34; ++j) {
+          const float x0 = j < 32 ? s[4 * j] : st[4 * (j - 32)], x1 = j < 32 ? s[4 * j + 1] : st[4 * (j - 32) + 1];
+          const float x2 = j < 32 ? s[4 * j + 2] : st[4 * (j - 32) + 2], x3 = j < 32 ? s[4 * j + 3] : st[4 * (j - 32) + 3];
+          const float p0 = ex2_approx((x0 - mx0) * kExpScale), p1 = ex2_approx((x1 - mx0) * kExpScale);
+          const float p2 = ex2_approx((x2 - mx1) * kExpScale), p3 = ex2_approx((x3 - mx1) * kExpScale);
+          sum0 += p0 + p1;
+          sum1 += p2 + p3;
+          const int c = j >> 1, h = (j & 1) * 2;
+          split_pair(p0, p1, ph_[4 * c + h], pl_[4 * c + h]);
+          split_pair(p2, p3, ph_[4 * c + h + 1], pl_[4 * c + h + 1]);
+        }
+#pragma unroll
+        for (int off = 1; off <= 2; off <<= 1) {
+          sum0 += __shfl_xor_sync(0xffffffffu, sum0, off);
+          sum1 += __shfl_xor_sync(0xffffffffu, sum1, off);
+        }
+        if (u == 0) {
+          mbar_wait(&tail.v_full, ph);
+          if (stamp && it < kStampItems) STAMP(3 + 4 * it);
+        }
+        float o[32];
+        acc_fence(o);
+        wgmma_fence();
+#pragma unroll
+        for (int c = 0; c < kKeys / 16; ++c) {
+          const uint32_t ah[4] = {ph_[4 * c], ph_[4 * c + 1], ph_[4 * c + 2], ph_[4 * c + 3]};
+          const uint64_t dvh = wgmma_desc_mnmajor_sw128(vh + c * 16 * kRow);
+          wgmma_rs_n64_bf16_tb(o, ah, dvh, c != 0 ? 1u : 0u);
+          if (passes == 3) {
+            const uint32_t al[4] = {pl_[4 * c], pl_[4 * c + 1], pl_[4 * c + 2], pl_[4 * c + 3]};
+            wgmma_rs_n64_bf16_tb(o, ah, wgmma_desc_mnmajor_sw128(vl + c * 16 * kRow), 1u);
+            wgmma_rs_n64_bf16_tb(o, al, dvh, 1u);
+          }
+        }
+        wgmma_commit();
+        wgmma_wait<0>();
+        acc_fence(o);
+        if (u == 1) {
+          __syncwarp();
+          if (lane == 0) mbar_arrive(&tail.v_empty);
+        }
+        if (passes == 3 && nitem < items) load_q_frag(qa_l, qkv_lo + qnext);
+        const float inv0 = 1.0f / sum0, inv1 = 1.0f / sum1;
+        const int tok0 = qt * 64 + wl * 16 + (lane >> 2);
+        const size_t o0 = (size_t)(row0 + tok0) * kDim + head * kHd + 2 * (lane & 3);
+        const size_t o1 = o0 + (size_t)8 * kDim;
+#pragma unroll
+        for (int j = 0; j < 8; ++j) {
+          uint32_t h, l;
+          split_pair(o[4 * j] * inv0, o[4 * j + 1] * inv0, h, l);
+          *reinterpret_cast<uint32_t*>(out_hi + o0 + 8 * j) = h;
+          *reinterpret_cast<uint32_t*>(out_lo + o0 + 8 * j) = l;
+          split_pair(o[4 * j + 2] * inv1, o[4 * j + 3] * inv1, h, l);
+          *reinterpret_cast<uint32_t*>(out_hi + o1 + 8 * j) = h;
+          *reinterpret_cast<uint32_t*>(out_lo + o1 + 8 * j) = l;
         }
       }
-      sj[i] = key < kTok ? acc : -INFINITY;
-      mx = fmaxf(mx, sj[i]);
+      if (stamp && it < kStampItems) STAMP(4 + 4 * it);
     }
-#pragma unroll
-    for (int off = 16; off > 0; off >>= 1) mx = fmaxf(mx, __shfl_xor_sync(0xffffffffu, mx, off));
-    float sum = 0.f;
-#pragma unroll
-    for (int i = 0; i < 9; ++i) {
-      const int key = lane + 32 * i;
-      const float pj = key < kTok ? ex2_approx((sj[i] - mx) * kExpScale) : 0.f;
-      sum += pj;
-      if (key < kKeys) s_p[key] = pj;
-    }
-#pragma unroll
-    for (int off = 16; off > 0; off >>= 1) sum += __shfl_xor_sync(0xffffffffu, sum, off);
-    __syncwarp();
-    mbar_wait(&tail.v_full, 0);
-    float o0[4] = {0.f, 0.f, 0.f, 0.f}, o1[4] = {0.f, 0.f, 0.f, 0.f};
-#pragma unroll 8
-    for (int key = 0; key < 256; ++key) {
-      const float2 vv = ld_pair_sw128(sV[0], vlo, key, 2 * lane);
-      const float pj = s_p[key];
-      o0[key & 3] = fmaf(pj, vv.x, o0[key & 3]);
-      o1[key & 3] = fmaf(pj, vv.y, o1[key & 3]);
-    }
-    {
-      const float2 vv = ld_pair_sw128(sV[0], vlo, 256, 2 * lane);
-      o0[0] = fmaf(s_p[256], vv.x, o0[0]);
-      o1[0] = fmaf(s_p[256], vv.y, o1[0]);
-    }
-    const float o0s = (o0[0] + o0[1]) + (o0[2] + o0[3]), o1s = (o1[0] + o1[1]) + (o1[2] + o1[3]);
-    const float inv = 1.0f / sum;
-    uint32_t h, l;
-    split_pair(o0s * inv, o1s * inv, h, l);
-    const size_t oo = (size_t)(row0 + 256) * kDim + head * kHd + 2 * lane;
-    *reinterpret_cast<uint32_t*>(out_hi + oo) = h;
-    *reinterpret_cast<uint32_t*>(out_lo + oo) = l;
-    }
-  } else {
-    const int wg = warp >> 2, wl = warp & 3;
-    const uint32_t kh = smem_u32(sK[0]), kl = smem_u32(sK[1]), vh = smem_u32(sV[0]), vl = smem_u32(sV[1]);
-    mbar_wait(&tail.qk_full, 0);
-    if (threadIdx.x == 0) STAMP(1);
-    for (int qt = wg; qt < kQTiles; qt += 2) {
-      const uint32_t qh = smem_u32(sQ[0] + qt * 64 * kRow), ql = smem_u32(sQ[1] + qt * 64 * kRow);
-      float s[128], st[8];
-      acc_fence(s); acc_fence(st);
-      wgmma_fence();
-#pragma unroll
-      for (int pass = 0; pass < passes; ++pass) {
-        const uint32_t a = pass == 2 ? ql : qh, b = pass == 1 ? kl : kh;
-#pragma unroll
-        for (int k16 = 0; k16 < 4; ++k16) {
-          const uint32_t acc = (pass | k16) != 0 ? 1u : 0u;
-          const uint64_t da = wgmma_desc_kmajor<kRow>(a + k16 * 32);
-          wgmma_ss_n256_bf16(s, da, wgmma_desc_kmajor<kRow>(b + k16 * 32), acc);
-          wgmma_ss_n16_bf16(st, da, wgmma_desc_kmajor<kRow>(b + 256 * kRow + k16 * 32), acc);
-        }
-      }
-      wgmma_commit();
-      wgmma_wait<0>();
-      acc_fence(s); acc_fence(st);
-      const bool key256 = (lane & 3) == 0;
-#pragma unroll
-      for (int i = 0; i < 8; ++i) if (!(key256 && (i & 1) == 0 && i < 4)) st[i] = -INFINITY;
-      float mx0 = fmaxf(st[0], st[1]), mx1 = fmaxf(st[2], st[3]);
-#pragma unroll
-      for (int j = 0; j < 32; ++j) {
-        mx0 = fmaxf(mx0, fmaxf(s[4 * j], s[4 * j + 1]));
-        mx1 = fmaxf(mx1, fmaxf(s[4 * j + 2], s[4 * j + 3]));
-      }
-#pragma unroll
-      for (int off = 1; off <= 2; off <<= 1) {
-        mx0 = fmaxf(mx0, __shfl_xor_sync(0xffffffffu, mx0, off));
-        mx1 = fmaxf(mx1, __shfl_xor_sync(0xffffffffu, mx1, off));
-      }
-      float sum0 = 0.f, sum1 = 0.f;
-      uint32_t ph[68], pl[68];
-#pragma unroll
-      for (int j = 0; j < 34; ++j) {
-        const float x0 = j < 32 ? s[4 * j] : st[4 * (j - 32)], x1 = j < 32 ? s[4 * j + 1] : st[4 * (j - 32) + 1];
-        const float x2 = j < 32 ? s[4 * j + 2] : st[4 * (j - 32) + 2], x3 = j < 32 ? s[4 * j + 3] : st[4 * (j - 32) + 3];
-        const float p0 = ex2_approx((x0 - mx0) * kExpScale), p1 = ex2_approx((x1 - mx0) * kExpScale);
-        const float p2 = ex2_approx((x2 - mx1) * kExpScale), p3 = ex2_approx((x3 - mx1) * kExpScale);
-        sum0 += p0 + p1;
-        sum1 += p2 + p3;
-        const int c = j >> 1, h = (j & 1) * 2;
-        split_pair(p0, p1, ph[4 * c + h], pl[4 * c + h]);
-        split_pair(p2, p3, ph[4 * c + h + 1], pl[4 * c + h + 1]);
-      }
-#pragma unroll
-      for (int off = 1; off <= 2; off <<= 1) {
-        sum0 += __shfl_xor_sync(0xffffffffu, sum0, off);
-        sum1 += __shfl_xor_sync(0xffffffffu, sum1, off);
-      }
-      if (qt == wg) mbar_wait(&tail.v_full, 0);
-      float o[32];
-      acc_fence(o);
-      wgmma_fence();
-#pragma unroll
-      for (int c = 0; c < kKeys / 16; ++c) {
-        const uint32_t ah[4] = {ph[4 * c], ph[4 * c + 1], ph[4 * c + 2], ph[4 * c + 3]};
-        const uint64_t dvh = wgmma_desc_mnmajor_sw128(vh + c * 16 * kRow);
-        wgmma_rs_n64_bf16_tb(o, ah, dvh, c != 0 ? 1u : 0u);
-        if (passes == 3) {
-          const uint32_t al[4] = {pl[4 * c], pl[4 * c + 1], pl[4 * c + 2], pl[4 * c + 3]};
-          wgmma_rs_n64_bf16_tb(o, ah, wgmma_desc_mnmajor_sw128(vl + c * 16 * kRow), 1u);
-          wgmma_rs_n64_bf16_tb(o, al, dvh, 1u);
-        }
-      }
-      wgmma_commit();
-      wgmma_wait<0>();
-      acc_fence(o);
-      const float inv0 = 1.0f / sum0, inv1 = 1.0f / sum1;
-      const int tok0 = qt * 64 + wl * 16 + (lane >> 2);
-      const size_t o0 = (size_t)(row0 + tok0) * kDim + head * kHd + 2 * (lane & 3);
-      const size_t o1 = o0 + (size_t)8 * kDim;
-#pragma unroll
-      for (int j = 0; j < 8; ++j) {
-        uint32_t h, l;
-        split_pair(o[4 * j] * inv0, o[4 * j + 1] * inv0, h, l);
-        *reinterpret_cast<uint32_t*>(out_hi + o0 + 8 * j) = h;
-        *reinterpret_cast<uint32_t*>(out_lo + o0 + 8 * j) = l;
-        split_pair(o[4 * j + 2] * inv1, o[4 * j + 3] * inv1, h, l);
-        *reinterpret_cast<uint32_t*>(out_hi + o1 + 8 * j) = h;
-        *reinterpret_cast<uint32_t*>(out_lo + o1 + 8 * j) = l;
-      }
-    }
-    if (lane == 0 && wl == 0) STAMP(2 + wg);
   }
 }
 
@@ -273,7 +402,7 @@
 
 cudaError_t launch_attention_tc(const CUtensorMap& hi128, const CUtensorMap& lo128, const CUtensorMap& hi16,
                                 const CUtensorMap& lo16, const uint16_t* qkv_hi, const uint16_t* qkv_lo, uint16_t* out_hi,
-                                uint16_t* out_lo, int b, int crop_stride, int passes, cudaStream_t s) {
+                                uint16_t* out_lo, int b, int crop_stride, int passes, int num_sms, cudaStream_t s) {
   static bool configured = false;
   if (!configured) {
     cudaError_t e = cudaFuncSetAttribute(attention_tc_kernel<3>, cudaFuncAttributeMaxDynamicSharedMemorySize, kSmem);
@@ -283,12 +412,12 @@
   }
   if (b <= 0) return cudaSuccess;
   const int items = b * kHeads;
-  const dim3 grid(items);
+  const dim3 grid(items < num_sms ? items : num_sms);
   auto qh = reinterpret_cast<const __nv_bfloat16*>(qkv_hi), ql = reinterpret_cast<const __nv_bfloat16*>(qkv_lo);
   auto oh = reinterpret_cast<__nv_bfloat16*>(out_hi), ol = reinterpret_cast<__nv_bfloat16*>(out_lo);
   if (passes == 3)
-    return launch_ex(attention_tc_kernel<3>, grid, dim3(kThreads), kSmem, s, 1, true, hi128, lo128, hi16, lo16, qh, ql, oh, ol, crop_stride);
-  return launch_ex(attention_tc_kernel<1>, grid, dim3(kThreads), kSmem, s, 1, true, hi128, lo128, hi16, lo16, qh, ql, oh, ol, crop_stride);
-}
-
-}
+    return launch_ex(attention_tc_kernel<3>, grid, dim3(kThreads), kSmem, s, 1, true, hi128, lo128, hi16, lo16, qh, ql, oh, ol, crop_stride, items);
+  return launch_ex(attention_tc_kernel<1>, grid, dim3(kThreads), kSmem, s, 1, true, hi128, lo128, hi16, lo16, qh, ql, oh, ol, crop_stride, items);
+}
+
+}
diff --git a/gigapose_b200/csrc/wgmma.cuh b/gigapose_b200/csrc/wgmma.cuh
--- a/gigapose_b200/csrc/wgmma.cuh
+++ b/gigapose_b200/csrc/wgmma.cuh
@@ -83,6 +83,26 @@
       : "+f"(d[0]), "+f"(d[1]), "+f"(d[2]), "+f"(d[3]), "+f"(d[4]), "+f"(d[5]), "+f"(d[6]), "+f"(d[7]), "+f"(d[8]), "+f"(d[9]), "+f"(d[10]), "+f"(d[11]), "+f"(d[12]), "+f"(d[13]), "+f"(d[14]), "+f"(d[15]), "+f"(d[16]), "+f"(d[17]), "+f"(d[18]), "+f"(d[19]), "+f"(d[20]), "+f"(d[21]), "+f"(d[22]), "+f"(d[23]), "+f"(d[24]), "+f"(d[25]), "+f"(d[26]), "+f"(d[27]), "+f"(d[28]), "+f"(d[29]), "+f"(d[30]), "+f"(d[31]), "+f"(d[32]), "+f"(d[33]), "+f"(d[34]), "+f"(d[35]), "+f"(d[36]), "+f"(d[37]), "+f"(d[38]), "+f"(d[39]), "+f"(d[40]), "+f"(d[41]), "+f"(d[42]), "+f"(d[43]), "+f"(d[44]), "+f"(d[45]), "+f"(d[46]), "+f"(d[47]), "+f"(d[48]), "+f"(d[49]), "+f"(d[50]), "+f"(d[51]), "+f"(d[52]), "+f"(d[53]), "+f"(d[54]), "+f"(d[55]), "+f"(d[56]), "+f"(d[57]), "+f"(d[58]), "+f"(d[59]), "+f"(d[60]), "+f"(d[61]), "+f"(d[62]), "+f"(d[63]), "+f"(d[64]), "+f"(d[65]), "+f"(d[66]), "+f"(d[67]), "+f"(d[68]), "+f"(d[69]), "+f"(d[70]), "+f"(d[71]), "+f"(d[72]), "+f"(d[73]), "+f"(d[74]), "+f"(d[75]), "+f"(d[76]), "+f"(d[77]), "+f"(d[78]), "+f"(d[79]), "+f"(d[80]), "+f"(d[81]), "+f"(d[82]), "+f"(d[83]), "+f"(d[84]), "+f"(d[85]), "+f"(d[86]), "+f"(d[87]), "+f"(d[88]), "+f"(d[89]), "+f"(d[90]), "+f"(d[91]), "+f"(d[92]), "+f"(d[93]), "+f"(d[94]), "+f"(d[95]), "+f"(d[96]), "+f"(d[97]), "+f"(d[98]), "+f"(d[99]), "+f"(d[100]), "+f"(d[101]), "+f"(d[102]), "+f"(d[103]), "+f"(d[104]), "+f"(d[105]), "+f"(d[106]), "+f"(d[107]), "+f"(d[108]), "+f"(d[109]), "+f"(d[110]), "+f"(d[111]), "+f"(d[112]), "+f"(d[113]), "+f"(d[114]), "+f"(d[115]), "+f"(d[116]), "+f"(d[117]), "+f"(d[118]), "+f"(d[119]), "+f"(d[120]), "+f"(d[121]), "+f"(d[122]), "+f"(d[123]), "+f"(d[124]), "+f"(d[125]), "+f"(d[126]), "+f"(d[127])
       : "l"(da), "l"(db), "r"(scale_d));
 }
+__device__ __forceinline__ void wgmma_rs_n16_bf16(float (&d)[8], const uint32_t (&a)[4], uint64_t db, uint32_t scale_d) {
+  asm volatile(
+      "{\n\t.reg .pred p;\n\t"
+      "setp.ne.b32 p, %13, 0;\n\t"
+      "wgmma.mma_async.sync.aligned.m64n16k16.f32.bf16.bf16 "
+      "{%0, %1, %2, %3, %4, %5, %6, %7}, "
+      "{%8, %9, %10, %11}, %12, p, 1, 1, 0;\n\t}"
+      : "+f"(d[0]), "+f"(d[1]), "+f"(d[2]), "+f"(d[3]), "+f"(d[4]), "+f"(d[5]), "+f"(d[6]), "+f"(d[7])
+      : "r"(a[0]), "r"(a[1]), "r"(a[2]), "r"(a[3]), "l"(db), "r"(scale_d));
+}
+__device__ __forceinline__ void wgmma_rs_n256_bf16(float (&d)[128], const uint32_t (&a)[4], uint64_t db, uint32_t scale_d) {
+  asm volatile(
+      "{\n\t.reg .pred p;\n\t"
+      "setp.ne.b32 p, %133, 0;\n\t"
+      "wgmma.mma_async.sync.aligned.m64n256k16.f32.bf16.bf16 "
+      "{%0, %1, %2, %3, %4, %5, %6, %7, %8, %9, %10, %11, %12, %13, %14, %15, %16, %17, %18, %19, %20, %21, %22, %23, %24, %25, %26, %27, %28, %29, %30, %31, %32, %33, %34, %35, %36, %37, %38, %39, %40, %41, %42, %43, %44, %45, %46, %47, %48, %49, %50, %51, %52, %53, %54, %55, %56, %57, %58, %59, %60, %61, %62, %63, %64, %65, %66, %67, %68, %69, %70, %71, %72, %73, %74, %75, %76, %77, %78, %79, %80, %81, %82, %83, %84, %85, %86, %87, %88, %89, %90, %91, %92, %93, %94, %95, %96, %97, %98, %99, %100, %101, %102, %103, %104, %105, %106, %107, %108, %109, %110, %111, %112, %113, %114, %115, %116, %117, %118, %119, %120, %121, %122, %123, %124, %125, %126, %127}, "
+      "{%128, %129, %130, %131}, %132, p, 1, 1, 0;\n\t}"
+      : "+f"(d[0]), "+f"(d[1]), "+f"(d[2]), "+f"(d[3]), "+f"(d[4]), "+f"(d[5]), "+f"(d[6]), "+f"(d[7]), "+f"(d[8]), "+f"(d[9]), "+f"(d[10]), "+f"(d[11]), "+f"(d[12]), "+f"(d[13]), "+f"(d[14]), "+f"(d[15]), "+f"(d[16]), "+f"(d[17]), "+f"(d[18]), "+f"(d[19]), "+f"(d[20]), "+f"(d[21]), "+f"(d[22]), "+f"(d[23]), "+f"(d[24]), "+f"(d[25]), "+f"(d[26]), "+f"(d[27]), "+f"(d[28]), "+f"(d[29]), "+f"(d[30]), "+f"(d[31]), "+f"(d[32]), "+f"(d[33]), "+f"(d[34]), "+f"(d[35]), "+f"(d[36]), "+f"(d[37]), "+f"(d[38]), "+f"(d[39]), "+f"(d[40]), "+f"(d[41]), "+f"(d[42]), "+f"(d[43]), "+f"(d[44]), "+f"(d[45]), "+f"(d[46]), "+f"(d[47]), "+f"(d[48]), "+f"(d[49]), "+f"(d[50]), "+f"(d[51]), "+f"(d[52]), "+f"(d[53]), "+f"(d[54]), "+f"(d[55]), "+f"(d[56]), "+f"(d[57]), "+f"(d[58]), "+f"(d[59]), "+f"(d[60]), "+f"(d[61]), "+f"(d[62]), "+f"(d[63]), "+f"(d[64]), "+f"(d[65]), "+f"(d[66]), "+f"(d[67]), "+f"(d[68]), "+f"(d[69]), "+f"(d[70]), "+f"(d[71]), "+f"(d[72]), "+f"(d[73]), "+f"(d[74]), "+f"(d[75]), "+f"(d[76]), "+f"(d[77]), "+f"(d[78]), "+f"(d[79]), "+f"(d[80]), "+f"(d[81]), "+f"(d[82]), "+f"(d[83]), "+f"(d[84]), "+f"(d[85]), "+f"(d[86]), "+f"(d[87]), "+f"(d[88]), "+f"(d[89]), "+f"(d[90]), "+f"(d[91]), "+f"(d[92]), "+f"(d[93]), "+f"(d[94]), "+f"(d[95]), "+f"(d[96]), "+f"(d[97]), "+f"(d[98]), "+f"(d[99]), "+f"(d[100]), "+f"(d[101]), "+f"(d[102]), "+f"(d[103]), "+f"(d[104]), "+f"(d[105]), "+f"(d[106]), "+f"(d[107]), "+f"(d[108]), "+f"(d[109]), "+f"(d[110]), "+f"(d[111]), "+f"(d[112]), "+f"(d[113]), "+f"(d[114]), "+f"(d[115]), "+f"(d[116]), "+f"(d[117]), "+f"(d[118]), "+f"(d[119]), "+f"(d[120]), "+f"(d[121]), "+f"(d[122]), "+f"(d[123]), "+f"(d[124]), "+f"(d[125]), "+f"(d[126]), "+f"(d[127])
+      : "r"(a[0]), "r"(a[1]), "r"(a[2]), "r"(a[3]), "l"(db), "r"(scale_d));
+}
 __device__ __forceinline__ void wgmma_rs_n64_bf16_tb(float (&d)[32], const uint32_t (&a)[4], uint64_t db, uint32_t scale_d) {
   asm volatile(
       "{\n\t.reg .pred p;\n\t"
```

Result: no change. 807.2 (median of 6 runs) (+0.9%).
